# PacificBiosciences/trgt

Hardware: AMD Instinct MI355X
Metric: loci/s (higher is better)
Workload: dtype u8/u16 (WFA) + f64 (HMM); 1 GPU; BASELINE configs[1]: 10000 synthetic single-motif STR loci per GPU (motif 3-6 bp, allele <= 200 bp), 30 reads/locus HiFi-like, 10% truncated reads (SURVEY.md Appendix E), seed 20250509; contexts_per_gpu=4, loci_per_gpu=10000, reads_per_locus=30, parallelism=loci sharded across 1 GPU(s), no collective

## Files before the change

### trgt_amd/csrc/common.hpp

```cpp
#pragma once
#include <hip/hip_runtime.h>

#include <cstdarg>
#include <cstdint>
#include <cstdio>
#include <cstring>
#include <ctime>
#include <algorithm>
#include <mutex>
#include <string>
#include <vector>

#include "../../include/trgt_hip.h"

#ifdef TRGT_DEV_BUILD
#define TRGT_DEV_ENV(name) getenv(name)
#else
#define TRGT_DEV_ENV(name) ((const char*)nullptr)
#endif

struct trgt_knobs {
  int filter_force = 0;
  int flank_threads = 256;
  int heavy_band = 96;
  int heavy_threads = 0;
  int band_threads = 64;
  int win_threads = 64;
  int win_segments = 8;
  bool win_lds = false;
  bool band_lds = false;
  int grid_per_cu = 0;
  int filter_per_cu = 0;
  bool one_launch = false;
  bool no_spec = false;
  bool no_window = false;
  bool early_adaptive = true;
  bool no_heavy_window = false;
  bool no_sibling_rule = false;
  bool no_settled_sibling_rule = false;
  bool no_lcs_rule = false;
  bool no_indel_shortcut = false;
  bool no_hamming = false;
  bool no_filter = false;
  bool one_stream = false;
  bool host_genotyper = false;
  bool no_early = false;
  bool stage_lock = false;
  bool host_hmm_lists = false;
  bool debug = false;
  bool hmm_resolve_one_wg = false;
  bool wfa_no_wave_variant = false;
  bool wfa_no_stage = false;
  bool filter_side = false;
  bool filter_serial = false;
  bool filter_one_launch = false;
  bool no_long_window = false;
  bool no_long_filter = false;
  bool no_lean = false;
  bool lean_mid_tier = false;
  int lean_chunk = 0;
  bool no_zero_arena = false;
  bool hmm_ppl_per_class = false;
  bool hmm_ppl_wide = false;
  bool hmm_trace_wide = false;
  bool hmm_ppl_serial = false;
  bool lean_one_tier = false;
  bool no_lds_wfa = true;
  int lds_wfa_kb = 7;
  int lds_wfa_seq = 768;
  int sens_bialign_min_len = -1;
  bool sens_cons_unidir = false;
  bool sens_ward_ties = false;
  bool sens_lw_order = false;
  bool hmm_no_dedupe = false;
  bool hmm_no_long_tb = false;
  int hmm_long_wgs = 4;
  bool hmm_no_ppl = false;
  bool hmm_four_rounds = false;
  bool hmm_lds_fill = false;
  int cluster_arena_kb = 0;
  int repair_arena_kb = 0;
  bool host_cluster = false;
  bool host_purity = false;
  bool host_repair = false;
  bool split_hmm = false;
  int repair_blocks = 2048;
  int repair_max_seg = 0;
  bool timeline = false;
  bool skip_bt = false;
};

enum FlankRoute {
  FR_SIZE_TAG = 0,
  FR_SIZE_SNV,
  FR_CLUSTER_TAG,
  FR_CLUSTER_SNV,
  FR_CLUSTER_DEEP_TAG,
  FR_CLUSTER_DEEP_SNV,
  FR_N
};
struct FlankRouteState { bool on = false; int64_t stats[4] = {0, 0, 0, 0}; };

struct trgt_hip_ctx {
  trgt_knobs knobs;
  int device = -1;
  hipStream_t stream = nullptr;
  bool own_stream = false;
  int stream_priority = 0;
  bool in_pool = false;
  std::string err;
  uint64_t ws_limit = 32ull << 30;
  int32_t cluster_max_reads = 256;
  int32_t size_max_reads = 256;
  int64_t size_deep_stats[4] = {0, 0, 0, 0};
  FlankRouteState route[FR_N];
  double meth_ms[2] = {0, 0};
  double plot_ms[2] = {0, 0};
  int num_cus = 256;
  int band_occ = 0;
  struct Buf { void* p = nullptr; size_t cap = 0; };
  std::vector<Buf> pool;
  bool timing = false;
  double k_ms[TRGT_K_COUNT] = {};
  int64_t k_launches[TRGT_K_COUNT] = {};
  int64_t k_cells[TRGT_K_COUNT] = {};
  struct Pending { int k; hipEvent_t a, b; };
  std::vector<Pending> pending;
  std::vector<hipEvent_t> retired_events;
  void* zero_arena = nullptr; size_t zero_cap = 0, zero_used = 0, zero_dirty = 0; bool zero_on = false;
  void* wfa_cells_cur[3] = {nullptr, nullptr, nullptr};
  void* last_wfa_cells_dev = nullptr;
// ... 105 lines not shown
  S_HMM_EDIT, S_HMM_MAXD, S_HMM_PLEN, S_HMM_VISITS, S_HMM_LONG, S_HMM_MOTIFS,
  S_HMM_B_BASE, S_HMM_B_LAST = S_HMM_B_BASE + (S_HMM_MOTIFS - S_HMM_SEQ),
  S_WFA_SEQ, S_WFA_JOBS, S_WFA_WS, S_WFA_STATUS, S_WFA_SCORE, S_WFA_NMATCH, S_WFA_SPAN, S_WFA_CIGAR, S_WFA_CLEN, S_WFA_OPS,
  S_WFA_OLEN, S_WFA_COUNTER, S_WFA_CELLS, S_WFA_WS_B, S_WFA_COUNTER_B, S_WFA_CELLS_B, S_WFA_POFF, S_WFA_PACKED, S_WFA_RETRY, S_WFA_RETRY_B, S_WFA_WS_C, S_WFA_COUNTER_C, S_WFA_CELLS_C, S_WFA_RETRY_C, S_WFA_MID, S_WFA_MID_B, S_WFA_MID_C,
  S_FS_FLANK, S_FS_READS, S_FS_JOBS, S_FS_POS, S_FS_LIST, S_FS_COUNT, S_FS_OUT0, S_FS_OUT1, S_FS_HIT0, S_FS_HIT1,
  S_FS_WFAJOBS, S_FS_WFAJOBS_LONG, S_FS_KEEPJOBS, S_PF_READS0, S_PF_READS1, S_PF_FLANK0, S_PF_FLANK1, S_READS_PACKED, S_READS_EXPANDED, S_FLT_COUNTER, S_FLT_CELLS, S_FLT_COUNTER_B, S_FLT_CELLS_B, S_LW_FIRST, S_LW_SUB, S_LW_PARENT, S_LW_SUBKEEP, S_LW_JOBKEEP, S_LW_KEPT, S_LW_COUNT, S_FLT_SEQ, S_FLT_JOBS, S_FLT_SCORE, S_FLT_BOUND, S_FLT_KEEP, S_FS_WINJOBS, S_FS_RESTJOBS, S_FS_SCORE, S_FS_SPAN, S_FS_NMATCH, S_FS_HEAVY, S_FS_NOSEED, S_FS_BANDJOBS, S_FS_HRESTJOBS, S_FS_BSCORE, S_FS_LONGNOSEED, S_LW_SUBBAND, S_LW_JOBBEST, S_LW_JOBREJ, S_LW_BANDJOBS, S_LW_RESTJOBS, S_LW_BSCORE,
  S_LOCUS_0, S_LOCUS_1, S_LOCUS_2, S_LOCUS_3, S_LOCUS_4, S_LOCUS_5, S_LOCUS_6, S_LOCUS_7,
  S_GT_LRB, S_GT_PLOIDY, S_GT_TR, S_GT_TROFF, S_GT_TRLEN, S_GT_ALOFF, S_GT_ALCAP, S_GT_NEED, S_GT_NAL, S_GT_BLOB, S_GT_ALEN, S_GT_CI, S_GT_NSP,
  S_GT_CLS, S_GT_RANK, S_GT_NSPAN, S_GT_TOFF, S_GT_PACKED, S_GT_GENO,
  S_HMM_BUILD,
  S_VOTE_GROUPS, S_VOTE_SCRATCH, S_VOTE_OUT, S_VOTE_LEN,
  S_RP_GROUPS, S_RP_JOBS, S_RP_LOCI, S_RP_PEND, S_RP_CIGAR, S_RP_CLEN, S_RP_VOUT, S_RP_VLEN, S_RP_VSCR, S_RP_COUNTS,
  S_CL_LIST, S_CL_MOFF, S_CL_COUNTS, S_CL_REC, S_CL_CLS, S_CL_ESCORE, S_CL_GMAT, S_CL_EDJOBS, S_CL_JOBS, S_CL_GROUPS, S_CL_ED2JOBS, S_CL_ESCORE2, S_CL_CIGAR, S_CL_CLEN,
  S_CL_VOUT, S_CL_VLEN, S_CL_VSCR,
  S_INF_SRC, S_INF_DESC, S_INF_DST, S_INF_STATUS, S_INF_COUNTER,
  S_ZERO_ARENA,
  S_DEFL_SCRATCH,
  S_PUR_SLAB, S_PUR_CNT, S_PUR_RQ,
  S_CLD_LIST, S_CLD_LAST = S_CLD_LIST + (S_CL_VSCR - S_CL_LIST),
  S_CLD_SEL,
  S_GSD_LIST,
  S_GT_HP,
  S_SNV_SO, S_SNV_EO, S_SNV_MM, S_SNV_MMOFF, S_SNV_READ,
  S_SNV_DEEP,
  S_CLF_COUNTS,
  S_CLF_PEND,
  S_CLDF_COUNTS, S_CLDF_PEND,
  S_FS_SETTLED, S_FS_FILTERJOBS,
  S_FS_BANDFALL, S_LW_BANDFALL,
  S_METH_READS, S_METH_CALLS, S_METH_JOBS, S_METH_LOCI, S_METH_LEVEL, S_METH_LEN, S_METH_FLAG, S_METH_OUT, S_METH_NREADS, S_METH_PERREAD,
  S_PLOT_IN, S_PLOT_PATH, S_PLOT_HMMOUT, S_PLOT_WORK, S_PLOT_WFAOUT, S_PLOT_PSEG, S_PLOT_NPSEG, S_PLOT_RSEG, S_PLOT_NRSEG, S_PLOT_BPROJ, S_PLOT_SCORE, S_PLOT_POFF, S_PLOT_PACKED,
  S_COUNT
};
enum PinSlot { P_SPAN_S = 0, P_SPAN_E, P_HIT_L, P_HIT_R, P_CELLS, P_HMM_SEQ, P_HMM_SEQ_B, P_HMM_JOBS, P_HMM_JOBS_B, P_SEG0, P_SEG_META, P_GT_NEED, P_GT_NAL, P_GT_ALEN, P_GT_CI, P_GT_NSP, P_GT_CLS,
               P_GT_RANK, P_GT_NSPAN, P_GT_TOFF, P_GT_PACKED, P_HMM_BUILD, P_PUR_JOBS, P_COUNT };

inline int dev_get(trgt_hip_ctx* c, int slot, size_t bytes, void** out) {
  if ((int)c->pool.size() < S_COUNT) c->pool.resize(S_COUNT);
  auto& b = c->pool[slot];
  if (bytes == 0) bytes = 16;
  if (b.cap < bytes) {
    if (b.p) { TRGT_HIP_TRY(c, hipFree(b.p)); b.p = nullptr; b.cap = 0; }
    size_t want = bytes + bytes / 8 + 256;
    if (c->knobs.debug && want > ((size_t)256 << 20)) fprintf(stderr, "[mem] slot %d: %.2f GB\n", slot, (double)want / (double)(1ull << 30));
    if (want >= ((size_t)64 << 20)) {
      size_t free_b = 0, total_b = 0;
      if (hipMemGetInfo(&free_b, &total_b) == hipSuccess) {
        const size_t reserve = (size_t)1 << 30;
        if (free_b < want || free_b - want < reserve)
          return fail(c, TRGT_ERR_NOMEM, "%zu bytes of device memory wanted, %zu free: less than 1 GB would be left for the runtime (fewer contexts per GPU, or a smaller trgt_hip_set_workspace_limit)", want, free_b);
      } else (void)hipGetLastError();
    }
    hipError_t e = hipMalloc(&b.p, want);
    if (e != hipSuccess) {
      (void)hipGetLastError();
      b.p = nullptr;
      return fail(c, TRGT_ERR_NOMEM, "hipMalloc(%zu bytes) failed: %s", want, hipGetErrorString(e));
    }
    b.cap = want;
  }
  *out = b.p;
  return TRGT_OK;
}

inline int pin_get(trgt_hip_ctx* c, int slot, size_t bytes, void** out) {
  if ((int)c->pinned.size() < P_COUNT) c->pinned.resize(P_COUNT);
  auto& b = c->pinned[slot];
  if (bytes == 0) bytes = 16;
  if (b.cap < bytes) {
    if (b.p) { TRGT_HIP_TRY(c, hipHostFree(b.p)); b.p = nullptr; b.cap = 0; }
    const size_t want = bytes + bytes / 4 + 4096;
    hipError_t e = hipHostMalloc(&b.p, want, hipHostMallocDefault);
    if (e != hipSuccess) {
      (void)hipGetLastError();
      b.p = nullptr;
      return fail(c, TRGT_ERR_NOMEM, "hipHostMalloc(%zu bytes) failed: %s", want, hipGetErrorString(e));
    }
    b.cap = want;
  }
  *out = b.p;
  return TRGT_OK;
}

constexpr size_t ZERO_ARENA_BYTES = 2u << 20;
static __global__ void zero_arena_kernel(uint4* __restrict__ p, size_t n16) {
  for (size_t i = (size_t)blockIdx.x * blockDim.x + threadIdx.x; i < n16; i += (size_t)gridDim.x * blockDim.x) p[i] = make_uint4(0u, 0u, 0u, 0u);
}
inline int zero_begin(trgt_hip_ctx* c) {
  c->zero_on = false;
  if (c->knobs.no_zero_arena) return TRGT_OK;
  void* p = nullptr;
  if (int rc = dev_get(c, S_ZERO_ARENA, ZERO_ARENA_BYTES, &p)) return rc;
  const bool fresh = p != c->zero_arena;
  c->zero_arena = p; c->zero_cap = ZERO_ARENA_BYTES;
  const size_t dirty = fresh ? ZERO_ARENA_BYTES : std::min(ZERO_ARENA_BYTES, (std::max(c->zero_dirty, c->zero_used) + 4095) & ~(size_t)4095);
  if (dirty) {
    const size_t n16 = dirty / 16;
    hipLaunchKernelGGL(zero_arena_kernel, dim3((unsigned)std::min<size_t>(64, (n16 + 255) / 256)), dim3(256), 0, c->stream, (uint4*)p, n16);
    TRGT_HIP_TRY(c, hipGetLastError());
  }
  c->zero_used = 0; c->zero_dirty = 0; c->zero_on = true;
  c->wfa_cells_cur[0] = c->wfa_cells_cur[1] = c->wfa_cells_cur[2] = nullptr;
  return TRGT_OK;
}
inline void zero_end(trgt_hip_ctx* c) {
  if (c->zero_on) { c->zero_dirty = std::max(c->zero_dirty, c->zero_used); c->zero_on = false; }
  c->wfa_cells_cur[0] = c->wfa_cells_cur[1] = c->wfa_cells_cur[2] = nullptr;
}
inline void* zero_take(trgt_hip_ctx* c, size_t bytes) {
  if (!c->zero_on) return nullptr;
  const size_t need = (bytes + 63) & ~(size_t)63;
  if (c->zero_used + need > c->zero_cap) return nullptr;
  void* p = (uint8_t*)c->zero_arena + c->zero_used;
  c->zero_used += need;
  return p;
}
inline int dev_get_zeroed(trgt_hip_ctx* c, int slot, size_t bytes, void** out, hipStream_t stream) {
  if (void* z = zero_take(c, bytes)) { *out = z; return TRGT_OK; }
  if (int rc = dev_get(c, slot, bytes, out)) return rc;
  TRGT_HIP_TRY(c, hipMemsetAsync(*out, 0, bytes, stream));
  return TRGT_OK;
}

constexpr size_t H2D_KERNEL_MAX = 8u << 20;
static __global__ void h2d_copy_kernel(uint8_t* __restrict__ dst, const uint8_t* __restrict__ src, size_t bytes) {
  const size_t i = (size_t)blockIdx.x * blockDim.x + threadIdx.x, n = (size_t)gridDim.x * blockDim.x;
  if ((((uintptr_t)dst | (uintptr_t)src) & 15u) == 0) {
    const size_t n16 = bytes >> 4;
    for (size_t k = i; k < n16; k += n) reinterpret_cast<uint4*>(dst)[k] = reinterpret_cast<const uint4*>(src)[k];
    for (size_t k = (n16 << 4) + i; k < bytes; k += n) dst[k] = src[k];
  } else for (size_t k = i; k < bytes; k += n) dst[k] = src[k];
}
inline bool is_pinned_host_ptr(const void* p) {
  hipPointerAttribute_t at;
  if (hipPointerGetAttributes(&at, p) != hipSuccess) { (void)hipGetLastError(); return false; }
  return at.type == hipMemoryTypeHost;
}
inline int d2h(trgt_hip_ctx* c, void* dst, const void* src, size_t bytes, hipStream_t stream) {
  if (bytes == 0) return TRGT_OK;
  if (is_pinned_host_ptr(dst)) { TRGT_HIP_TRY(c, hipMemcpyAsync(dst, src, bytes, hipMemcpyDeviceToHost, stream)); return TRGT_OK; }
  const size_t need = (bytes + 63) & ~(size_t)63;
  trgt_hip_ctx::D2hChunk* ch = nullptr;
  for (auto& k : c->d2h_chunks) if (k.cap - k.used >= need) { ch = &k; break; }
  if (!ch) {
    trgt_hip_ctx::D2hChunk k;
    k.cap = std::max<size_t>(need, (size_t)4 << 20);
    if (hipHostMalloc(&k.p, k.cap, hipHostMallocDefault) != hipSuccess) { (void)hipGetLastError(); return fail(c, TRGT_ERR_NOMEM, "hipHostMalloc(%zu bytes) failed", k.cap); }
    c->d2h_chunks.push_back(k);
    ch = &c->d2h_chunks.back();
  }
  void* staged = (uint8_t*)ch->p + ch->used;
  ch->used += need;
  TRGT_HIP_TRY(c, hipMemcpyAsync(staged, src, bytes, hipMemcpyDeviceToHost, stream));
  c->d2h_pending.push_back({dst, staged, bytes, stream});
  return TRGT_OK;
}
inline hipError_t stream_wait(trgt_hip_ctx* c, hipStream_t stream) {
  const hipError_t e = stream_wait(stream);
  if (c->d2h_pending.empty()) return e;
  size_t kept = 0;
  for (auto& q : c->d2h_pending) {
    if (q.stream == stream) { if (e == hipSuccess) std::memcpy(q.dst, q.staged, q.bytes); }
    else c->d2h_pending[kept++] = q;
  }
  c->d2h_pending.resize(kept);
  if (kept == 0) {
// ... 178 lines not shown
```

### trgt_amd/csrc/ctx.hip

```cpp
#include "common.hpp"
#include "host_pool.hpp"

static std::string g_create_err;

#include <malloc.h>
static void tune_malloc_once() {
  static std::once_flag once;
  std::call_once(once, [] {
    const char* e = getenv("TRGT_MALLOC_TUNE");
    const int mode = e && *e ? atoi(e) : 1;
    if (mode <= 0) return;
    (void)mallopt(M_MMAP_THRESHOLD, 32 << 20);
    (void)mallopt(M_TRIM_THRESHOLD, 1 << 30);
    (void)mallopt(M_TOP_PAD, 64 << 20);
    if (mode >= 2) (void)mallopt(M_MMAP_MAX, 0);
  });
}

namespace trgt {
static thread_local int g_next_stream_priority = 0;
static thread_local bool g_next_in_pool = false;
void ctx_next_stream_priority(int p) { g_next_stream_priority = p; }
void ctx_next_in_pool(bool on) { g_next_in_pool = on; }
hipError_t make_stream(trgt_hip_ctx* c, hipStream_t* s) {
  return c->stream_priority ? hipStreamCreateWithPriority(s, hipStreamNonBlocking, c->stream_priority) : hipStreamCreateWithFlags(s, hipStreamNonBlocking);
}
hipError_t make_side_stream(trgt_hip_ctx* c, hipStream_t* s) {
  if (c->in_pool) return make_stream(c, s);
  int lo = 0, hi = 0;
  if (hipDeviceGetStreamPriorityRange(&lo, &hi) != hipSuccess || lo <= hi) { (void)hipGetLastError(); return make_stream(c, s); }
  const int base = c->stream_priority;
  const int side = base != hi ? hi : hi + 1;
  return hipStreamCreateWithPriority(s, hipStreamNonBlocking, side);
}
}

extern "C" {

int trgt_hip_abi_version(void) { return TRGT_HIP_ABI_VERSION; }

int trgt_hip_create(int device, trgt_hip_ctx** out) {
  if (!out) return TRGT_ERR_INVALID;
  *out = nullptr;
  int n = 0;
  hipError_t e = hipGetDeviceCount(&n);
  if (e != hipSuccess || n <= 0) {
    (void)hipGetLastError();
    g_create_err = "no HIP device visible (libtrgt_hip has no CPU fallback)";
    return TRGT_ERR_NO_DEVICE;
  }
  if (device < 0 || device >= n) { g_create_err = "device ordinal out of range"; return TRGT_ERR_INVALID; }
  e = hipSetDevice(device);
  if (e != hipSuccess) { g_create_err = hipGetErrorString(e); return TRGT_ERR_HIP; }
  hipDeviceProp_t prop;
  e = hipGetDeviceProperties(&prop, device);
  if (e != hipSuccess) { g_create_err = hipGetErrorString(e); return TRGT_ERR_HIP; }
  if (std::strncmp(prop.gcnArchName, "gfx950", 6) != 0) {
    g_create_err = std::string("device is ") + prop.gcnArchName + ", this library carries gfx950 code only";
    return TRGT_ERR_NO_DEVICE;
  }
  tune_malloc_once();
  trgt_hip_ctx* c = new trgt_hip_ctx();
  {
    trgt_knobs& k = c->knobs;
    auto num = [](const char* name, int dflt) { const char* e = getenv(name); return e && *e ? atoi(e) : dflt; };
    auto flag = [](const char* name) { const char* e = getenv(name); return e != nullptr && *e != 0 && std::strcmp(e, "0") != 0; };
#ifdef TRGT_DEV_BUILD
#define DEV_FLAG(name) flag(name)
#define DEV_NUM(name, dflt) num(name, dflt)
#else
#define DEV_FLAG(name) false
#define DEV_NUM(name, dflt) (dflt)
#endif
    (void)num; (void)flag;
    k.flank_threads = DEV_NUM("TRGT_FLANK_THREADS", k.flank_threads); k.heavy_threads = DEV_NUM("TRGT_HEAVY_THREADS", 0); k.heavy_band = std::max(0, std::min(num("TRGT_HEAVY_BAND", k.heavy_band), 256));
    k.win_threads = DEV_NUM("TRGT_WIN_THREADS", k.win_threads); { const int bt = DEV_NUM("TRGT_BAND_THREADS", k.band_threads); k.band_threads = bt == 128 || bt == 256 ? bt : 64; } k.win_segments = DEV_NUM("TRGT_WIN_SEGMENTS", k.win_segments); k.win_lds = DEV_FLAG("TRGT_WIN_LDS"); k.band_lds = DEV_FLAG("TRGT_BAND_LDS");
    k.grid_per_cu = DEV_NUM("TRGT_WFA_GRID_PER_CU", 0); k.filter_per_cu = DEV_NUM("TRGT_FILTER_PER_CU", 0);
    k.one_launch = DEV_FLAG("TRGT_WFA_ONE_LAUNCH"); k.no_spec = DEV_FLAG("TRGT_WFA_NO_SPEC"); k.no_window = flag("TRGT_WFA_NO_WINDOW"); k.no_hamming = flag("TRGT_NO_HAMMING"); k.no_indel_shortcut = flag("TRGT_NO_INDEL_SHORTCUT"); k.no_heavy_window = DEV_FLAG("TRGT_NO_HEAVY_WINDOW"); k.no_sibling_rule = DEV_FLAG("TRGT_NO_SIBLING_RULE"); k.no_settled_sibling_rule = DEV_FLAG("TRGT_NO_SETTLED_SIBLING_RULE"); k.no_lcs_rule = DEV_FLAG("TRGT_NO_LCS_RULE"); { const char* e = TRGT_DEV_ENV("TRGT_EARLY_ADAPTIVE"); if (e && *e) k.early_adaptive = std::strcmp(e, "0") != 0; }
    k.no_filter = flag("TRGT_WFA_NO_FILTER"); k.one_stream = DEV_FLAG("TRGT_FLANK_ONE_STREAM"); k.host_genotyper = flag("TRGT_HOST_GENOTYPER"); k.host_hmm_lists = DEV_FLAG("TRGT_HOST_HMM_LISTS"); k.no_early = flag("TRGT_WFA_NO_EARLY"); k.stage_lock = flag("TRGT_STAGE_LOCK"); k.no_long_filter = flag("TRGT_NO_LONG_FILTER"); k.no_long_window = DEV_FLAG("TRGT_NO_LONG_WINDOW"); k.filter_force = DEV_NUM("TRGT_FILTER_FORCE", 0); k.filter_one_launch = DEV_FLAG("TRGT_FILTER_ONE_LAUNCH"); k.filter_serial = DEV_FLAG("TRGT_FILTER_SERIAL"); k.filter_side = DEV_FLAG("TRGT_FILTER_SIDE"); k.wfa_no_stage = DEV_FLAG("TRGT_WFA_NO_STAGE"); k.wfa_no_wave_variant = DEV_FLAG("TRGT_WFA_NO_WAVE_VARIANT"); k.hmm_resolve_one_wg = DEV_FLAG("TRGT_HMM_RESOLVE_ONE_WG"); k.debug = flag("TRGT_WFA_DEBUG");
    k.timeline = flag("TRGT_TIMELINE");
    k.host_repair = flag("TRGT_HOST_REPAIR"); k.host_cluster = flag("TRGT_HOST_CLUSTER"); k.host_purity = DEV_FLAG("TRGT_HOST_PURITY"); k.cluster_arena_kb = num("TRGT_CLUSTER_ARENA_KB", 0); k.repair_arena_kb = num("TRGT_REPAIR_ARENA_KB", 0); k.hmm_lds_fill = DEV_FLAG("TRGT_HMM_LDS_FILL"); k.hmm_four_rounds = DEV_FLAG("TRGT_HMM_FOUR_ROUNDS"); k.hmm_no_ppl = flag("TRGT_HMM_NO_PPL"); k.hmm_long_wgs = std::max(1, std::min(DEV_NUM("TRGT_HMM_LONG_WGS", k.hmm_long_wgs), 16)); k.hmm_no_long_tb = flag("TRGT_HMM_NO_LONG_TB"); k.hmm_no_dedupe = flag("TRGT_HMM_NO_DEDUPE"); k.repair_max_seg = num("TRGT_REPAIR_MAX_SEG", k.repair_max_seg); k.split_hmm = DEV_FLAG("TRGT_SPLIT_HMM"); k.repair_blocks = DEV_NUM("TRGT_REPAIR_BLOCKS", k.repair_blocks);
    k.no_lean = flag("TRGT_WFA_NO_LEAN"); k.lean_one_tier = DEV_FLAG("TRGT_WFA_LEAN_ONE_TIER"); k.lean_mid_tier = DEV_FLAG("TRGT_WFA_LEAN_MID_TIER"); k.lean_chunk = DEV_NUM("TRGT_LEAN_CHUNK", 0); k.no_zero_arena = flag("TRGT_NO_ZERO_ARENA"); k.hmm_ppl_serial = DEV_FLAG("TRGT_HMM_PPL_SERIAL"); k.hmm_ppl_wide = DEV_FLAG("TRGT_HMM_PPL_WIDE"); k.hmm_trace_wide = DEV_FLAG("TRGT_HMM_TRACE_WIDE"); k.hmm_ppl_per_class = DEV_FLAG("TRGT_HMM_PPL_PER_CLASS");
    k.no_lds_wfa = !DEV_FLAG("TRGT_WFA_LDS"); k.lds_wfa_kb = DEV_NUM("TRGT_WFA_LDS_KB", k.lds_wfa_kb); k.lds_wfa_seq = DEV_NUM("TRGT_WFA_LDS_SEQ", k.lds_wfa_seq);
#ifdef TRGT_DEV_BUILD
    k.sens_bialign_min_len = num("TRGT_SENS_BIALIGN_MIN_LEN", -1); k.sens_cons_unidir = flag("TRGT_SENS_CONS_UNIDIR"); k.sens_ward_ties = flag("TRGT_SENS_WARD_TIES"); k.sens_lw_order = flag("TRGT_SENS_LW_ORDER");
    k.skip_bt = flag("TRGT_DBG_SKIP_BT");
#endif
  }
  c->device = device;
  c->num_cus = prop.multiProcessorCount;
  c->stream_priority = trgt::g_next_stream_priority;
  c->in_pool = trgt::g_next_in_pool;
  e = trgt::make_stream(c, &c->stream);
  if (e != hipSuccess) { g_create_err = hipGetErrorString(e); delete c; return TRGT_ERR_HIP; }
  c->own_stream = true;
  c->pool.resize(trgt::S_COUNT);
  *out = c;
  return TRGT_OK;
}

void trgt_hip_destroy(trgt_hip_ctx* c) {
  if (!c) return;
  (void)hipSetDevice(c->device);
  (void)trgt::stream_wait(c, c->stream);
  if (c->stream2) { (void)trgt::stream_wait(c, c->stream2); (void)hipStreamDestroy(c->stream2); }
  if (c->ev_upload) (void)hipEventDestroy(c->ev_upload);
  if (c->stream_copy) { (void)trgt::stream_wait(c, c->stream_copy); (void)hipStreamDestroy(c->stream_copy); }
  for (auto& st : c->staged) if (st.ready) (void)hipEventDestroy(st.ready);
  for (int i = 0; i < 6; ++i) {
    if (c->hmm_side[i]) { (void)trgt::stream_wait(c, c->hmm_side[i]); (void)hipStreamDestroy(c->hmm_side[i]); }
    if (c->hmm_join[i]) (void)hipEventDestroy(c->hmm_join[i]);
  }
  for (int i = 0; i < 2; ++i) if (c->hmm_fork[i]) (void)hipEventDestroy(c->hmm_fork[i]);
  for (int b = 0; b < 2; ++b)
    for (int k = 0; k < 4; ++k) {
      for (int g = 0; g < 3; ++g) {
        if (c->hmm_ppl_side[b][k][g]) { (void)trgt::stream_wait(c, c->hmm_ppl_side[b][k][g]); (void)hipStreamDestroy(c->hmm_ppl_side[b][k][g]); }
        if (c->hmm_ppl_join[b][k][g]) (void)hipEventDestroy(c->hmm_ppl_join[b][k][g]);
      }
      if (c->hmm_ppl_fork[b][k]) (void)hipEventDestroy(c->hmm_ppl_fork[b][k]);
    }
  if (c->ev_scan) (void)hipEventDestroy(c->ev_scan);
  if (c->ev_heavy) (void)hipEventDestroy(c->ev_heavy);
  if (c->ev_hwin) (void)hipEventDestroy(c->ev_hwin);
  if (c->stream_hmm) (void)hipStreamDestroy(c->stream_hmm);
  if (c->stream_flt) (void)hipStreamDestroy(c->stream_flt);
  if (c->ev_flt_a) (void)hipEventDestroy(c->ev_flt_a);
  if (c->ev_flt_b) (void)hipEventDestroy(c->ev_flt_b);
  if (c->ev_gt) (void)hipEventDestroy(c->ev_gt);
  if (c->ev_rp) (void)hipEventDestroy(c->ev_rp);
  delete static_cast<trgt::HostPool*>(c->host_pool);
  for (auto& b : c->h2d_stage) if (b.p) (void)hipHostFree(b.p);
  for (auto& k : c->d2h_chunks) if (k.p) (void)hipHostFree(k.p);
  for (auto& b : c->pinned)
    if (b.p) (void)hipHostFree(b.p);
  trgt::resolve_timing(c);
  for (auto& b : c->pool)
    if (b.p) (void)hipFree(b.p);
  trgt::resolve_timing(c);
  for (hipEvent_t e : c->retired_events) (void)hipEventDestroy(e);
  if (c->own_stream && c->stream) (void)hipStreamDestroy(c->stream);
  delete c;
}

const char* trgt_hip_last_error(const trgt_hip_ctx* c) { return c ? c->err.c_str() : g_create_err.c_str(); }

int trgt_hip_set_stream(trgt_hip_ctx* c, void* s) {
  if (!c) return TRGT_ERR_INVALID;
  (void)hipSetDevice(c->device);
  TRGT_HIP_TRY(c, trgt::stream_wait(c, c->stream));
  if (c->own_stream && c->stream) (void)hipStreamDestroy(c->stream);
  if (s == nullptr) {
    TRGT_HIP_TRY(c, trgt::make_stream(c, &c->stream));
    c->own_stream = true;
  } else {
    c->stream = (hipStream_t)s;
    c->own_stream = false;
  }
  return TRGT_OK;
// ... 38 lines not shown
```

### trgt_amd/csrc/hmm.hip

```cpp
#include <algorithm>
#include <type_traits>
#include <cmath>
#include <limits>
#include <thread>

#include "common.hpp"

namespace trgt {


}
#include <memory>

#include "hmm_host.hpp"
namespace trgt {

struct HmmJobDev {
  uint32_t set, seq_len, job_index, path_cap;
  uint64_t seq_off, bp_off, path_off, span_off, count_off, visit_off;
  uint64_t map_off;
};

static inline uint64_t align_up(uint64_t v, uint64_t a) { return (v + a - 1) / a * a; }

// ... 1332 lines not shown
#pragma unroll
  for (int c = 1; c < HMM_SLOT_CLASSES; ++c) k += i >= a.class_begin[c] ? 1u : 0u;
  return k;
}
__global__ void __launch_bounds__(256) hmm_resolve_count_kernel(const HmmResolveAllArgs a) {
  const uint32_t i = blockIdx.x * 256u + threadIdx.x;
  const int lane = (int)(threadIdx.x & 63u);
  uint32_t v = 0, key = 0;
  if (i < a.n) {
    const uint32_t slot = a.cand[i].job_index, l = slot >> 1, al = slot & 1u;
    const bool on = !a.skip_locus[l] && (int32_t)al < a.n_alleles[l];
    if (!on) { a.n_spans[slot] = 0; a.purity[slot] = __builtin_nan(""); }
    v = on ? a.allele_len[slot] + 1u : 0u;
    if (a.dup) {
      uint8_t d = 0;
      if (on && al == 1u && i > 0 && a.cand[i - 1].job_index == slot - 1u && a.allele_len[slot - 1u] == a.allele_len[slot]) {
        const uint8_t* p = a.seq_blob + a.cand[i - 1].seq_off; const uint8_t* q = a.seq_blob + a.cand[i].seq_off;
        const uint32_t n = a.allele_len[slot];
        uint64_t diff = 0;
        uint32_t t = 0;
        for (; t + 8 <= n; t += 8) { uint64_t x, y; __builtin_memcpy(&x, p + t, 8); __builtin_memcpy(&y, q + t, 8); diff |= x ^ y; }
        for (; t < n; ++t) diff |= (uint64_t)(p[t] ^ q[t]);
        d = diff == 0 ? 1 : 0;
      }
      a.dup[i] = d;
      if (d) v = 0;
    }
    a.verdict[i] = v;
    if (v) { const uint32_t b = (v - 1u) >> a.len_shift; key = hmm_class_of(a, i) * 64u + (63u - (b < 63u ? b : 63u)); }
  }
  uint32_t rank, count, leader;
  hmm_wave_keys(v != 0u, key, lane, rank, count, leader);
  if (v && rank == 0u) atomicAdd(&a.hist[key], count);
}
__global__ void __launch_bounds__(256) hmm_resolve_scatter_kernel(const HmmResolveAllArgs a) {
  __shared__ uint32_t base[HMM_RESOLVE_KEYS];
  for (uint32_t t = threadIdx.x; t < (uint32_t)HMM_RESOLVE_KEYS; t += 256) base[t] = a.hist[t];
  __syncthreads();
  if (threadIdx.x < (uint32_t)HMM_SLOT_CLASSES) {
    uint32_t run = 0;
    for (int b = 0; b < 64; ++b) { const uint32_t h = base[threadIdx.x * 64 + b]; base[threadIdx.x * 64 + b] = run; run += h; }
    if (blockIdx.x == 0) a.n_jobs[threadIdx.x] = run;
  }
  __syncthreads();
  const uint32_t i = blockIdx.x * 256u + threadIdx.x;
  const int lane = (int)(threadIdx.x & 63u);
  const uint32_t v = i < a.n ? a.verdict[i] : 0u;
  uint32_t key = 0, k = 0;
  if (v) { k = hmm_class_of(a, i); const uint32_t b = (v - 1u) >> a.len_shift; key = k * 64u + (63u - (b < 63u ? b : 63u)); }
  uint32_t rank, count, leader;
  hmm_wave_keys(v != 0u, key, lane, rank, count, leader);
  uint32_t at = 0;
  if (v && rank == 0u) at = atomicAdd(&a.taken[key], count);
  at = (uint32_t)__shfl((int)at, (int)leader);
  if (!v) return;
  HmmJobDev jd = a.cand[i];
  jd.seq_len = v - 1u;
  a.jobs[a.class_begin[k] + base[key] + at + rank] = jd;
}

__global__ void __launch_bounds__(256) hmm_dup_copy_kernel(const HmmJobDev* __restrict__ cand, uint32_t n, const uint8_t* __restrict__ dup, const HmmSetDev* __restrict__ sets,
                                                           int32_t* __restrict__ spans3, uint32_t* __restrict__ n_spans, uint32_t* __restrict__ counts, double* __restrict__ purity) {
  const uint32_t i = blockIdx.x * 256u + threadIdx.x;
  if (i >= n || !dup[i]) return;
  const HmmJobDev a = cand[i - 1], b = cand[i];
  const uint32_t ns = n_spans[a.job_index];
  n_spans[b.job_index] = ns; purity[b.job_index] = purity[a.job_index];
  for (uint32_t k = 0; k < 3 * ns; ++k) spans3[3 * b.span_off + k] = spans3[3 * a.span_off + k];
  const uint32_t nm = sets[b.set].n_blocks - 1;
  for (uint32_t k = 0; k < nm; ++k) counts[b.count_off + k] = counts[a.count_off + k];
}

__global__ void hmm_pack_spans_kernel(const int32_t* __restrict__ spans3, const uint64_t* __restrict__ job_span_off,
                                      const uint32_t* __restrict__ n_spans, const uint64_t* __restrict__ packed_off,
                                      int32_t* __restrict__ packed, uint64_t n_jobs) {
  const uint64_t j = (uint64_t)blockIdx.x * blockDim.x + threadIdx.x;
  if (j >= n_jobs) return;
  const int32_t* src = spans3 + 3 * job_span_off[j];
  int32_t* dst = packed + 3 * packed_off[j];
  for (uint32_t i = 0; i < 3 * n_spans[j]; ++i) dst[i] = src[i];
}

__global__ void __launch_bounds__(1024) hmm_span_prefix_kernel(const uint32_t* __restrict__ n_spans, uint64_t* __restrict__ off, uint64_t n) {
  __shared__ uint64_t part[1024];
  const uint32_t t = threadIdx.x;
  const uint64_t per = (n + 1023) / 1024, b = t * per < n ? t * per : n, e = b + per < n ? b + per : n;
  uint64_t sum = 0;
  for (uint64_t i = b; i < e; ++i) sum += n_spans[i];
  part[t] = sum;
  __syncthreads();
  if (t == 0) { uint64_t run = 0; for (int i = 0; i < 1024; ++i) { const uint64_t v = part[i]; part[i] = run; run += v; } off[n] = run; }
  __syncthreads();
  uint64_t run = part[t];
  for (uint64_t i = b; i < e; ++i) { off[i] = run; run += n_spans[i]; }
}


#include "hmm_batch.hpp"

}

using namespace trgt;

extern "C" uint64_t trgt_hmm_path_capacity(uint32_t seq_len, uint32_t max_motif_len) {
  if (seq_len == 0) return 1;
  return (uint64_t)(seq_len + 2) * (max_motif_len + 4) + 8;
}

extern "C" int trgt_hmm_models_check(trgt_hip_ctx* c, int32_t n_sets, const uint8_t* motif_blob, const uint32_t* motif_off,
                                     const uint32_t* set_motif_begin, int64_t* n_diff) {
  if (!c || !n_diff) return TRGT_ERR_INVALID;
  *n_diff = -1;
  HmmModels dev, host;
  int rc = hmm_models_on_device(c, n_sets, motif_blob, motif_off, set_motif_begin, dev, c->stream, nullptr);
  if (rc) return fail(c, rc, "%s", dev.err.empty() ? trgt_hip_last_error(c) : dev.err.c_str());
  rc = hmm_build_models(n_sets, motif_blob, motif_off, set_motif_begin, host);
  if (rc) return fail(c, rc, "%s", host.err.c_str());
  std::vector<uint8_t> got((size_t)dev.blob_bytes);
  if (dev.blob_bytes) { const int d2h_rc = trgt::d2h(c, got.data(), dev.d_blob, (size_t)dev.blob_bytes, c->stream); if (d2h_rc) return d2h_rc; }
  TRGT_HIP_TRY(c, trgt::stream_wait(c, c->stream));
  int64_t diff = dev.blob_bytes > host.blob.size() ? (int64_t)(dev.blob_bytes - host.blob.size()) : (int64_t)(host.blob.size() - dev.blob_bytes);
  const size_t n = std::min((size_t)dev.blob_bytes, host.blob.size());
  for (size_t i = 0; i < n; ++i) diff += got[i] != host.blob[i];
  const uint8_t *a = (const uint8_t*)dev.sets.data(), *b = (const uint8_t*)host.sets.data();
  for (size_t i = 0; i < sizeof(HmmSetDev) * (size_t)n_sets; ++i) diff += a[i] != b[i];
  *n_diff = diff;
  return TRGT_OK;
}

extern "C" int trgt_hmm_batch(trgt_hip_ctx* c, int32_t n_sets, const uint8_t* motif_blob, const uint32_t* motif_off,
                              const uint32_t* set_motif_begin, int64_t n_jobs, const uint32_t* job_set,
                              const uint8_t* seq_blob, const uint64_t* seq_off, const uint32_t* seq_len, uint16_t* path,
                              const uint64_t* path_off, uint32_t* path_len, int32_t* spans3, const uint64_t* span_off,
                              uint32_t* n_spans, uint32_t* motif_counts, const uint64_t* count_off, double* purity,
                              int32_t* edit_dist, int32_t* max_dist) {
  HmmBatchIO io;
  io.n_sets = n_sets; io.motif_blob = motif_blob; io.motif_off = motif_off; io.set_motif_begin = set_motif_begin;
  io.n_jobs = n_jobs; io.job_set = job_set; io.seq_blob = seq_blob; io.seq_off = seq_off; io.seq_len = seq_len;
  io.path = path; io.path_off = path_off; io.path_len = path_len; io.spans3 = spans3; io.span_off = span_off; io.n_spans = n_spans;
  io.motif_counts = motif_counts; io.count_off = count_off; io.purity = purity; io.edit_dist = edit_dist; io.max_dist = max_dist;
  return hmm_batch_impl(c, nullptr, io);
}
```

### trgt_amd/csrc/locus.hip

```cpp
#include <algorithm>
#include <array>
#include <chrono>
#include <cmath>
#include <cstddef>
#include <cstdlib>
#include <functional>
#include <optional>
#include <thread>

#include "hmm_host.hpp"
#include "host_pool.hpp"
#include "locus_gt.hpp"
#include "locus_purity.hpp"
#include "locus_cluster_dev.hpp"
#include "locus_cluster_deep.hpp"
#include "locus_cluster_flank.hpp"
#include "locus_gt_deep.hpp"
#include "locus_cluster_flank_deep.hpp"
#include "wfa_host.hpp"

namespace trgt {

namespace {

// ... 337 lines not shown
      }
      if (nc && (x != m_len[j] || y != bb_len[g])) return fail(c, TRGT_ERR_INVALID, "trgt_dev_consensus_vote: CIGAR of member %llu ends at (%llu, %llu), not at (%u, %u)", (unsigned long long)j, (unsigned long long)x, (unsigned long long)y, m_len[j], bb_len[g]);
      JobDev& jd = jobs[(size_t)j];
      jd.pat_off = bb_off[g]; jd.pat_len = bb_len[g]; jd.txt_off = m_off[j]; jd.txt_len = m_len[j]; jd.cigar_off = slot_words; jd.ops_off = 0; jd.out_index = (uint32_t)j; jd.pad = 0;
      po[(size_t)j] = bb_off[g]; pl[(size_t)j] = bb_len[g]; clen[(size_t)j] = (uint32_t)nc;
      slot_words += (uint64_t)bb_len[g] + m_len[j] + 1;
    }
  }
  first[(size_t)n_groups] = n_members;
  std::vector<uint32_t> slots((size_t)slot_words, 0xFFFFFFFFu);
  for (size_t j = 0; j < n_members; ++j) std::copy(cigar + cigar_first[j], cigar + cigar_first[j + 1], slots.begin() + (ptrdiff_t)jobs[j].cigar_off);
  int rc;
  void *d_seq = nullptr, *d_jobs = nullptr, *d_cig = nullptr, *d_clen = nullptr;
  if ((rc = dev_get(c, S_WFA_SEQ, (size_t)seq_bytes + 16, &d_seq)) || (rc = dev_get(c, S_WFA_JOBS, n_members * sizeof(JobDev), &d_jobs)) ||
      (rc = dev_get(c, S_WFA_CIGAR, (size_t)slot_words * 4 + 16, &d_cig)) || (rc = dev_get(c, S_WFA_CLEN, n_members * 4, &d_clen)))
    return rc;
  TRGT_HIP_TRY(c, hipMemcpyAsync(d_seq, seqs, (size_t)seq_bytes, hipMemcpyHostToDevice, c->stream));
  TRGT_HIP_TRY(c, hipMemcpyAsync(d_jobs, jobs.data(), n_members * sizeof(JobDev), hipMemcpyHostToDevice, c->stream));
  TRGT_HIP_TRY(c, hipMemcpyAsync(d_cig, slots.data(), (size_t)slot_words * 4, hipMemcpyHostToDevice, c->stream));
  TRGT_HIP_TRY(c, hipMemcpyAsync(d_clen, clen.data(), n_members * 4, hipMemcpyHostToDevice, c->stream));
  TRGT_HIP_TRY(c, trgt::stream_wait(c, c->stream));
  WfaOnDevice dev;
  dev.jobs = (const JobDev*)d_jobs; dev.cigar = (const uint32_t*)d_cig; dev.cigar_len = (const uint32_t*)d_clen; dev.seqs = (const uint8_t*)d_seq;
  std::vector<vote::Group> groups;
  std::vector<uint32_t> lens;
  std::vector<uint8_t> bytes;
  if ((rc = vote_groups(c, dev, po.data(), pl.data(), m_len, first, out_cap, count_on_device != 0, 0, groups, lens, bytes))) return rc;
  for (int64_t g = 0; g < n_groups; ++g) {
    out_len[g] = lens[(size_t)g];
    if (lens[(size_t)g] == 0xFFFFFFFFu) continue;
    const uint64_t room = out_off[g + 1] - out_off[g];
    std::memcpy(out_bytes + out_off[g], bytes.data() + groups[(size_t)g].out_off, (size_t)std::min<uint64_t>(room, lens[(size_t)g]));
  }
  return TRGT_OK;
}
#endif

#include "locus_cluster.hpp"

__global__ void repair_check_kernel(const gt::RepairBufs rp, uint64_t read_bytes) {
  const uint32_t nj = rp.counts[gt::RC_JOBS], ng = rp.counts[gt::RC_GROUPS];
  for (uint32_t j = blockIdx.x * blockDim.x + threadIdx.x; j < nj; j += gridDim.x * blockDim.x) {
    const JobDev jd = rp.jobs[j];
    const bool bad = jd.pat_len > rp.max_seg || jd.txt_len > rp.max_seg || jd.pat_off + jd.pat_len > read_bytes || jd.txt_off + jd.txt_len > read_bytes ||
                     jd.cigar_off + jd.pat_len + jd.txt_len + 1 > rp.cap_cigar || jd.out_index != j;
    if (bad) { atomicAdd(rp.counts + 10, 1u); rp.counts[11] = j; rp.counts[12] = jd.pat_len; rp.counts[13] = jd.txt_len; rp.counts[14] = jd.out_index; rp.counts[15] = (uint32_t)jd.cigar_off; }
  }
  if (blockIdx.x == 0 && threadIdx.x == 0 && (nj > rp.cap_jobs || ng > rp.cap_groups)) atomicAdd(rp.counts + 10, 1000000u);
}

static uint32_t* g_trace_dump = nullptr;
static uint32_t* repair_trace_buf() {
  if (!TRGT_DEV_ENV("TRGT_REPAIR_TRACE")) return nullptr;
  if (!g_trace_dump) (void)hipHostMalloc((void**)&g_trace_dump, 4096, hipHostMallocDefault);
  return g_trace_dump;
}
__global__ void repair_trace_kernel(const gt::RepairBufs rp, uint32_t* host) {
  if (threadIdx.x < gt::RC_WORDS) host[threadIdx.x] = __hip_atomic_load(rp.counts + threadIdx.x, __ATOMIC_RELAXED, __HIP_MEMORY_SCOPE_AGENT);
  if (threadIdx.x < 8) { const JobDev jd = rp.jobs[threadIdx.x]; uint32_t* h = host + 16 + 8 * threadIdx.x;
    h[0] = (uint32_t)jd.pat_off; h[1] = jd.pat_len; h[2] = (uint32_t)jd.txt_off; h[3] = jd.txt_len; h[4] = (uint32_t)jd.cigar_off; h[5] = jd.out_index; h[6] = (uint32_t)(jd.pat_off >> 32); h[7] = (uint32_t)(jd.txt_off >> 32); }
  __threadfence_system();
}
__global__ void zero_words_kernel(uint32_t* p, uint32_t n) { for (uint32_t i = threadIdx.x; i < n; i += blockDim.x) atomicExch(p + i, 0u); }

struct GatherArgs { const uint8_t* reads; const uint64_t* src_off; const uint64_t* dst_off; const uint32_t* len; uint64_t n; uint8_t* out; };
__global__ void gather_segments_kernel(const GatherArgs a) {
  const uint64_t s = (uint64_t)blockIdx.x * 4 + (threadIdx.x >> 6);
  if (s >= a.n) return;
  const uint8_t* __restrict__ src = a.reads + a.src_off[s];
  uint8_t* __restrict__ dst = a.out + a.dst_off[s];
  for (uint32_t i = threadIdx.x & 63; i < a.len[s]; i += 64) dst[i] = src[i];
}

inline int64_t now_ns() { return std::chrono::duration_cast<std::chrono::nanoseconds>(std::chrono::steady_clock::now().time_since_epoch()).count(); }

HostPool* host_pool(trgt_hip_ctx* c, int threads) {
  if (c->host_pool && c->host_pool_threads != threads) { delete static_cast<HostPool*>(c->host_pool); c->host_pool = nullptr; }
  if (!c->host_pool) { c->host_pool = new HostPool(threads); c->host_pool_threads = threads; }
  return static_cast<HostPool*>(c->host_pool);
}

struct CountCopy { const uint32_t* src1; uint32_t* dst1; uint32_t n1; const uint32_t* src2; uint32_t* dst2; uint32_t n2; const uint32_t* src3; uint32_t* dst3; uint32_t n3; };
__global__ void __launch_bounds__(1024) allele_prefix_kernel(const uint32_t* __restrict__ len, uint64_t* __restrict__ off, int64_t n, const CountCopy cc) {
  __shared__ uint64_t part[1024];
  const int t = threadIdx.x;
  if ((uint32_t)t < cc.n1) cc.dst1[t] = cc.src1 ? __hip_atomic_load(cc.src1 + t, __ATOMIC_RELAXED, __HIP_MEMORY_SCOPE_AGENT) : 0u;
  if ((uint32_t)t < cc.n2) cc.dst2[t] = cc.src2 ? __hip_atomic_load(cc.src2 + t, __ATOMIC_RELAXED, __HIP_MEMORY_SCOPE_AGENT) : 0u;
  if ((uint32_t)t < cc.n3) cc.dst3[t] = cc.src3 ? __hip_atomic_load(cc.src3 + t, __ATOMIC_RELAXED, __HIP_MEMORY_SCOPE_AGENT) : 0u;
  const int64_t per = (n + 1023) / 1024, b = t * per, e = b + per < n ? b + per : n;
  uint64_t sum = 0;
  for (int64_t i = b; i < e; ++i) sum += len[i];
  part[t] = sum;
  __syncthreads();
  if (t == 0) { uint64_t run = 0; for (int i = 0; i < 1024; ++i) { const uint64_t v = part[i]; part[i] = run; run += v; } off[n] = run; }
  __syncthreads();
  uint64_t run = part[t];
  for (int64_t i = b; i < e; ++i) { off[i] = run; run += len[i]; }
}
__global__ void allele_pack_kernel(const uint8_t* __restrict__ blob, const uint64_t* __restrict__ src_off, const uint32_t* __restrict__ len,
                                   const uint64_t* __restrict__ dst_off, uint8_t* __restrict__ packed, int64_t n) {
  const int64_t i = (int64_t)blockIdx.x * 4 + (threadIdx.x >> 6);
  if (i >= n) return;
  const uint8_t* s = blob + src_off[i];
  uint8_t* d = packed + dst_off[i];
  for (uint32_t b = threadIdx.x & 63; b < len[i]; b += 64) d[b] = s[b];
}

}
}

using namespace trgt;

extern "C" int32_t trgt_median_i32(const int32_t* data, int64_t n, float* out) {
  if (n < 0 || (n > 0 && !data) || !out) return TRGT_ERR_INVALID;
  if (n == 0) return 0;
  try { std::vector<int32_t> v(data, data + n); *out = median_f32(v); return 1; } catch (const std::exception&) { return TRGT_ERR_NOMEM; }
}

extern "C" void trgt_locus_default_params(trgt_locus_params* p) {
  if (!p) return;
  std::memset(p, 0, sizeof *p);
  p->flank_len = 250; p->min_flank_id_frac = 0.7; p->max_depth = 250; p->mism = 2; p->gapo = 5; p->gape = 1; p->host_threads = 0;
  p->min_read_qual = 0.98;
}

static std::mutex g_upload_mutex[16];
static hipStream_t g_upload_stream[16];
static hipStream_t bulk_upload_stream(trgt_hip_ctx* c) {
  static const bool shared = [] { const char* e = TRGT_DEV_ENV("TRGT_SHARED_UPLOAD_STREAM"); return !(e && *e == '0'); }();
  if (!shared) return c->stream_copy;
  const size_t d = (size_t)c->device % 16;
  if (!g_upload_stream[d] && hipStreamCreateWithFlags(&g_upload_stream[d], hipStreamNonBlocking) != hipSuccess) { (void)hipGetLastError(); return c->stream_copy; }
  return g_upload_stream[d];
}
static int issue_pending_uploads(trgt_hip_ctx* c) {
  bool any = false;
  for (auto& st : c->staged) any = any || (st.in_use && st.copy_pending);
  if (!any) return TRGT_OK;
  std::lock_guard<std::mutex> upload_lock(g_upload_mutex[(size_t)c->device % 16]);
  const hipStream_t up = bulk_upload_stream(c);
  for (auto& st : c->staged) {
    if (!st.in_use || !st.copy_pending) continue;
    st.copy_pending = false;
    if (st.d_reads) {
      static const size_t piece = [] { const char* e = TRGT_DEV_ENV("TRGT_UPLOAD_CHUNK_MB"); const long v = e && *e ? atol(e) : 32; return v > 0 ? (size_t)v << 20 : (size_t)0; }();
      const size_t total = (size_t)st.read_bytes;
      static const int kernel_wgs = [] { const char* e = TRGT_DEV_ENV("TRGT_UPLOAD_KERNEL"); return e && *e ? atoi(e) : 0; }();
      if (kernel_wgs > 0 && is_pinned_host_ptr(st.in->read_blob)) {
        hipLaunchKernelGGL(h2d_copy_kernel, dim3((unsigned)kernel_wgs), dim3(256), 0, up, const_cast<uint8_t*>(st.d_reads), st.in->read_blob, total);
        TRGT_HIP_TRY(c, hipGetLastError());
      } else
      for (size_t o = 0; o < total; o += piece ? piece : total) {
        const size_t n = piece ? std::min(piece, total - o) : total;
        TRGT_HIP_TRY(c, hipMemcpyAsync(const_cast<uint8_t*>(st.d_reads) + o, st.in->read_blob + o, n, hipMemcpyHostToDevice, up));
      }
    }
    if (st.d_flank) TRGT_HIP_TRY(c, hipMemcpyAsync(const_cast<uint8_t*>(st.d_flank), st.in->flank_blob, (size_t)st.flank_bytes, hipMemcpyHostToDevice, up));
    TRGT_HIP_TRY(c, hipEventRecord(st.ready, up));
  }
  return TRGT_OK;
}

static std::mutex g_stage_a_mutex[16];

__device__ __forceinline__ uint32_t bam4_pair_to_ascii(uint32_t b) {
  const uint64_t lo = 0x565352474d43413dull , hi = 0x4e42444b48595754ull ;
  const uint32_t a = b >> 4, z = b & 15u;
  const uint32_t ca = (uint32_t)(((a & 8u) ? hi : lo) >> (8 * (a & 7u))) & 0xFFu, cz = (uint32_t)(((z & 8u) ? hi : lo) >> (8 * (z & 7u))) & 0xFFu;
  return ca | (cz << 8);
}
__global__ void __launch_bounds__(256) expand_bam4_kernel(const uint8_t* __restrict__ packed, uint8_t* __restrict__ out, uint64_t n_bytes) {
  const uint64_t n16 = n_bytes / 16;
  for (uint64_t i = (uint64_t)blockIdx.x * blockDim.x + threadIdx.x; i < n16; i += (uint64_t)gridDim.x * blockDim.x) {
    const uint4 v = ((const uint4*)packed)[i];
    const uint32_t w[4] = {v.x, v.y, v.z, v.w};
    uint32_t o[8];
#pragma unroll
    for (int k = 0; k < 4; ++k) {
      o[2 * k] = bam4_pair_to_ascii(w[k] & 0xFFu) | (bam4_pair_to_ascii((w[k] >> 8) & 0xFFu) << 16);
      o[2 * k + 1] = bam4_pair_to_ascii((w[k] >> 16) & 0xFFu) | (bam4_pair_to_ascii(w[k] >> 24) << 16);
// ... 72 lines not shown

  trgt_hip_ctx* const c; const trgt_locus_params* const p; const trgt_locus_batch_in* in; trgt_locus_batch_out* const out;
  const uint8_t *staged_reads, *staged_flank; const hipEvent_t ready;
  const int64_t nl; int64_t nr = 0; int F = 0;
  bool done = false;
  trgt_locus_batch_in in_expanded; std::vector<uint64_t> expanded_off;
  bool reads_on_device = false, impure_filter = false, dev_gt = false, presel = false, flank_on = false, use_slots = false, dev_repair = false, split = false, small_gt = false;
  FlankMeta flank_meta{};
  bool zeroed = false;
  HmmPending *hmm_pending = nullptr, *hmm_pending2 = nullptr, *hmm_pendingB = nullptr;
  hipEvent_t evA = nullptr;
  std::unique_lock<std::mutex> stage_a_token;
  std::optional<StreamGuard> host_streams;
  HostPool* pool = nullptr;
  std::vector<uint64_t> piece_off; std::vector<uint32_t> read_locus, heavy_len;
  uint64_t flank_total = 0, read_total = 0, tr_total = 0, allele_total = 0, max_locus_reads = 0; uint32_t max_read_len = 0, heavy_tlen_max = 0;
  UploadBatch ub;
  const uint8_t *d_flank = nullptr, *d_reads = nullptr; const uint64_t *d_piece = nullptr, *d_roff = nullptr; const uint32_t *d_rlen = nullptr, *d_rloc = nullptr, *d_heavy = nullptr;
  void *d_ss = nullptr, *d_se = nullptr, *d_hl = nullptr, *d_hr = nullptr, *h_ss = nullptr, *h_se = nullptr, *h_hl = nullptr, *h_hr = nullptr, *h_cells = nullptr;
  Slab slab;
  size_t o_ss = 0, o_se = 0, o_hl = 0, o_hr = 0, o_need = 0, o_nal = 0, o_alen = 0, o_ci = 0, o_nsp = 0, o_cls = 0, o_rank = 0, o_nspan = 0, o_toff = 0, o_flip = 0, o_gsz = 0,
         o_rpc = 0, o_skipb = 0, o_clc = 0, o_cldc = 0, o_fdone = 0, o_cfc = 0, o_cfdc = 0;
  GtDev g; GtHost gh;
  ClPlan clp[2];
  std::vector<uint32_t>& cl_list = clp[0].list; std::vector<uint32_t>& cld_list = clp[1].list;
  uint32_t cld_no_room = 0;
  std::vector<uint32_t> gsd_list; const uint32_t* d_gsd_list = nullptr;
  gt::GtArgs ga; RepairDev rb;
  const uint32_t* cl_counts_dev[2] = {nullptr, nullptr};
  cld::DeepArgs da, ds;
  HmmModels models; HmmSlots hs;
  HmmBatchIO hmm_io(uint32_t* n_spans, double* purity) const {
    HmmBatchIO io;
    io.n_sets = (int32_t)nl; io.motif_blob = in->motif_blob; io.motif_off = in->motif_off; io.set_motif_begin = in->set_motif_begin;
    io.spans3 = out->spans3; io.span_off = out->span_off; io.n_spans = n_spans; io.motif_counts = out->motif_counts; io.count_off = out->count_off; io.purity = purity;
    return io;
  }
  HmmBatchIO hmm_list_io(const std::vector<uint32_t>& set, const void* blob, const std::vector<uint64_t>& off, const std::vector<uint32_t>& len, uint32_t* n_spans, double* purity) const {
    HmmBatchIO io = hmm_io(n_spans, purity);
    io.n_jobs = (int64_t)set.size(); io.job_set = set.data(); io.seq_blob = (const uint8_t*)blob; io.seq_off = off.data(); io.seq_len = len.data();
    return io;
  }
  hipStream_t upload_stream = nullptr;
  std::vector<uint8_t> slot_skip;
  std::vector<uint32_t> nsB; std::vector<double> puB;
  std::vector<uint32_t> job_set, seq_len, nsp; std::vector<uint64_t> seq_off, span_off, count_off; std::vector<int64_t> slot; std::vector<double> pur;
  std::vector<uint32_t> js2, sl2, ns2; std::vector<uint64_t> so2, spo2, co2; std::vector<double> pu2; std::vector<int64_t> slot2;
  bool outputs_ready = false;
  bool published = false, hmm1_done = false;
  std::vector<int64_t> R; int64_t nR = 0;
  std::vector<uint8_t> need_a;
  const int32_t *sp_s = nullptr, *sp_e = nullptr;
  std::vector<LocusWork> work; std::vector<uint64_t> sel_begin; std::vector<K> sel; std::vector<uint32_t> n_sel; std::vector<Scratch> scratch;
  std::vector<uint64_t> seg_src, seg_dst; std::vector<uint32_t> seg_len, seg_read; std::vector<const uint8_t*> seg_ptr;
  uint64_t n_seg = 0, seg_bytes = 0; void* h_seg = nullptr;
  std::vector<ClusterLocus> cl_loci; std::vector<std::vector<Seg>> cl_trs; std::vector<FlankRes> fres;
  bool tl_on = false;
  int64_t t0 = 0, tA = 0, tB = 0, tC = 0, tHost = 0, tw_a = 0, th_begin = 0, th0 = 0;
  int64_t stat_flank_jobs = 0, stat_flank_heavy = 0, stat_cons_jobs = 0, stat_spanning = 0, stat_hmm_jobs = 0, stat_ed_jobs = 0;

  LocusCall(trgt_hip_ctx* c_, const trgt_locus_params* p_, const trgt_locus_batch_in* in_, trgt_locus_batch_out* out_, const uint8_t* staged_reads_,
            const uint8_t* staged_flank_, hipEvent_t ready_)
      : c(c_), p(p_), in(in_), out(out_), staged_reads(staged_reads_), staged_flank(staged_flank_), ready(ready_), nl(in_->n_loci),
        stage_a_token(g_stage_a_mutex[(size_t)c_->device % 16], std::defer_lock), ub(c_, c_->stream) {}
  ~LocusCall() {
    host_streams.reset();
    if (stage_a_token.owns_lock()) stage_a_token.unlock();
    if (evA) (void)hipEventDestroy(evA);
    for (HmmPending* q : {hmm_pendingB, hmm_pending2, hmm_pending}) if (q) hmm_pending_free(q);
    if (zeroed) trgt::zero_end(c);
  }

  bool is_cluster(int64_t l) const { return in->genotyper && in->genotyper[l] == 1; }
  bool fits[FR_N] = {}, ran[FR_N] = {};
  void plan_routes();
  bool any_route_fits() const { return std::any_of(fits, fits + FR_N, [](bool b) { return b; }); }
  bool cluster_route_fits() const { return fits[FR_CLUSTER_TAG] || fits[FR_CLUSTER_SNV]; }
  bool deep_cluster_route_fits() const { return fits[FR_CLUSTER_DEEP_TAG] || fits[FR_CLUSTER_DEEP_SNV]; }
  bool snv_inputs_up() const { return fits[FR_SIZE_SNV] || fits[FR_CLUSTER_SNV] || fits[FR_CLUSTER_DEEP_SNV]; }
  bool tags_up() const { return fits[FR_SIZE_TAG] || fits[FR_CLUSTER_TAG] || fits[FR_CLUSTER_DEEP_TAG] || (snv_inputs_up() && in->hp_tag); }
  enum class GtForm { PLAIN, FLANK, SNV };
  GtForm gt_form() const { return fits[FR_SIZE_SNV] ? GtForm::SNV : fits[FR_SIZE_TAG] ? GtForm::FLANK : GtForm::PLAIN; }
  void launch_genotype_kernels(), launch_finish_kernels(const gt::FinishArgs& fa);
  void tally_route(FlankRoute r, const std::vector<uint32_t>* list, uint8_t snv, const uint8_t* fdone, const uint8_t* need);
  gt::GtFlankArgs flank_args() const { gt::GtFlankArgs fa; static_cast<gt::GtArgs&>(fa) = ga; fa.hp_tag = g.hp; fa.flank_done = (uint8_t*)slab.d(o_fdone); return fa; }
  gt::SnvArgs snv_args() const {
    gt::SnvArgs sa; static_cast<gt::GtFlankArgs&>(sa) = flank_args();
    sa.start_offset = g.so; sa.end_offset = g.eo; sa.mismatch_offsets = g.mm; sa.mismatch_off = g.mm_off; sa.snv_read = (uint8_t*)g.snv_read;
    sa.ln_match = std::log(0.9); sa.ln_mis = std::log(1.0 - 0.9); sa.ln2 = std::log(2.0); sa.tag_route = fits[FR_SIZE_TAG] ? 1 : 0;
    return sa;
  }
  gtd::DeepFlankArgs deep_flank_args() const { return gtd::DeepFlankArgs{ds, g.hp, (uint8_t*)slab.d(o_fdone)}; }
  gtd::DeepSnvArgs deep_snv_args() const {
    gtd::DeepSnvArgs da; static_cast<gtd::DeepFlankArgs&>(da) = deep_flank_args();
    const gt::SnvArgs sa = snv_args();
    da.start_offset = sa.start_offset; da.end_offset = sa.end_offset; da.mismatch_offsets = sa.mismatch_offsets; da.mismatch_off = sa.mismatch_off; da.snv_read = sa.snv_read;
    da.ln_match = sa.ln_match; da.ln_mis = sa.ln_mis; da.ln2 = sa.ln2; da.tag_route = sa.tag_route;
    da.prof = (uint64_t*)g.snv_prof; da.stage = (int32_t*)g.snv_stage; da.stage_cap = in->mismatch_off[nr];
    return da;
  }
  uint64_t& cell(int w) { return ((uint64_t*)h_cells)[w]; }
  void tl(const char* name) const { if (tl_on) fprintf(stderr, "[tl] %-28s %7.2f ms  ctx=%p\n", name, (double)(now_ns() - t0) / 1e6, (void*)c); }

  int check_args(), host_tables(), upload_tables(), plan_device_lists(), flush_uploads(), locate_flanks();
  int repair_buffers(), purity_chain(), size_genotyper(), repair_chain(), cluster_chain(int deep), enqueue_results();
  int wait_stage_a(), gather_host_segments(), host_front(), host_flank(), host_back(), host_stage_c(), collect_all();
  void stage_c_job_lists(), select_host_reads();
  void init_outputs();
  int collect_ab(), collect_hmm1(), hmm1_enqueue(), hmm1_once(), publish();
};
int LocusCall::check_args() {
  if (nl < 0) return fail(c, TRGT_ERR_INVALID, "trgt_locus_batch: negative n_loci");
  for (int64_t& v : c->size_deep_stats) v = 0;
  for (FlankRouteState& r : c->route) for (int64_t& v : r.stats) v = 0;
  if (nl == 0) { done = true; return TRGT_OK; }
  if (!in->flank_blob || !in->lf_off || !in->lf_len || !in->rf_off || !in->rf_len || !in->tr_blob || !in->tr_off || !in->tr_len ||
      !in->motif_blob || !in->motif_off || !in->set_motif_begin || !in->ploidy || !in->locus_read_begin || !in->read_blob ||
      !in->read_off || !in->read_len || !out->span_start || !out->span_end || !out->n_alleles || !out->allele_blob ||
      !out->allele_off || !out->allele_cap || !out->allele_len || !out->ci || !out->num_spanning || !out->classification ||
      !out->read_rank || !out->spans3 || !out->span_off || !out->n_spans || !out->motif_counts || !out->count_off || !out->purity)
    return fail(c, TRGT_ERR_INVALID, "trgt_locus_batch: null field");
  TRGT_HIP_TRY(c, hipSetDevice(c->device));
  zeroed = true;
  { const int zrc = trgt::zero_begin(c); if (zrc) return zrc; }
  F = p->flank_len;
  if (F <= 0) return fail(c, TRGT_ERR_INVALID, "trgt_locus_batch: flank_len must be positive");
  nr = (int64_t)in->locus_read_begin[nl];
  if (2 * nr > 0xFFFFFFF0ll) return fail(c, TRGT_ERR_UNSUPPORTED, "trgt_locus_batch: too many reads in one call");
  if (in->read_encoding != TRGT_READS_ASCII && in->read_encoding != TRGT_READS_BAM4) return fail(c, TRGT_ERR_INVALID, "trgt_locus_batch: read_encoding %d", in->read_encoding);
  if (in->read_encoding == TRGT_READS_BAM4 && nr > 0) {
    uint64_t packed_total = 0;
    expanded_off.resize((size_t)nr);
    for (int64_t r = 0; r < nr; ++r) {
      packed_total = std::max<uint64_t>(packed_total, in->read_off[r] + ((uint64_t)in->read_len[r] + 1) / 2);
      expanded_off[(size_t)r] = 2 * in->read_off[r];
    }
    const uint8_t* d_packed = nullptr;
    void* d_exp = nullptr;
    int erc;
    if (ready) TRGT_HIP_TRY(c, hipStreamWaitEvent(c->stream, ready, 0));
    if (staged_reads) d_packed = staged_reads;
    else if ((erc = dev_in(c, S_READS_PACKED, in->read_blob, (size_t)packed_total, &d_packed))) return erc;
    if ((erc = dev_get(c, S_READS_EXPANDED, 2 * (size_t)packed_total + 64, &d_exp))) return erc;
    const unsigned blocks = (unsigned)std::min<uint64_t>((uint64_t)c->num_cus * 16, packed_total / (16 * 256) + 1);
    hipLaunchKernelGGL(expand_bam4_kernel, dim3(blocks), dim3(256), 0, c->stream, d_packed, (uint8_t*)d_exp, packed_total);
    TRGT_HIP_TRY(c, hipGetLastError());
    in_expanded = *in;
    in_expanded.read_blob = (const uint8_t*)d_exp; in_expanded.read_off = expanded_off.data(); in_expanded.read_encoding = TRGT_READS_ASCII;
    in = &in_expanded;
    staged_reads = nullptr;
  }
  return TRGT_OK;
}
void LocusCall::init_outputs() {
  for (int64_t l = 0; l < nl; ++l) {
    out->n_alleles[l] = 0; out->allele_len[2 * l] = out->allele_len[2 * l + 1] = 0; out->num_spanning[2 * l] = out->num_spanning[2 * l + 1] = 0;
    if (out->gt_size) out->gt_size[2 * l] = out->gt_size[2 * l + 1] = 0;
    if (out->flipped) out->flipped[l] = 0;
  }
  for (int64_t r = 0; r < nr; ++r) { out->classification[r] = -1; out->read_rank[r] = -1; out->span_start[r] = out->span_end[r] = -1; }
  for (int64_t s = 0; s < 2 * nl; ++s) { out->n_spans[s] = 0; out->purity[s] = std::nan(""); }
}
int LocusCall::host_tables() {
  int threads = p->host_threads > 0 ? p->host_threads : (int)std::max(1u, std::thread::hardware_concurrency());
  threads = std::min(threads, !c->knobs.host_genotyper && !(p->min_read_qual < 0.9 && c->knobs.host_purity) ? 8 : 32);
  pool = host_pool(c, threads);
// ... 262 lines not shown
    da.c.g = ga; da.purity_on = 1; da.read_qual = pa.read_qual; da.pj_counter = pa.counter; da.pj = pa.jobs; da.pj_cap = pa.cap_jobs; da.purity = pa.purity;
    hipLaunchKernelGGL(cld::deep_select_kernel, dim3(da.c.n_list), dim3(cld::DW), 0, c->stream, da);
  }
  if (!gsd_list.empty()) {
    ds.c.g = ga; ds.purity_on = 1; ds.read_qual = pa.read_qual; ds.pj_counter = pa.counter; ds.pj = pa.jobs; ds.pj_cap = pa.cap_jobs; ds.purity = pa.purity;
    hipLaunchKernelGGL(cld::deep_select_kernel, dim3(ds.c.n_list), dim3(cld::DW), 0, c->stream, ds);
  }
  TRGT_HIP_TRY(c, hipGetLastError());
  *(uint32_t*)h_pj = 0;
  { const int d2h_rc = trgt::d2h(c, h_pj, pa.counter, 4, c->stream); if (d2h_rc) return d2h_rc; }
  tl_mark(c, "purity selection enqueued");
  init_outputs(); outputs_ready = true;
  const int64_t tw_p = now_ns();
  TRGT_HIP_TRY(c, trgt::stream_wait(c, c->stream));
  tA += now_ns() - tw_p;
  tl("purity jobs listed");
  const int64_t n_pj = (int64_t)std::min<uint32_t>(*(const uint32_t*)h_pj, pa.cap_jobs);
  if (n_pj > 0) {
    const pur::PurityJob* pj = pa.jobs;
    std::vector<uint32_t> pj_set((size_t)n_pj), pj_len((size_t)n_pj); std::vector<uint64_t> pj_off((size_t)n_pj), pj_cnt_off((size_t)n_pj);
    uint64_t cnt_total = 0;
    for (int64_t j = 0; j < n_pj; ++j) {
      if ((int64_t)pj[j].locus >= nl) return fail(c, TRGT_ERR_INVALID, "trgt_locus_batch: purity job %lld names locus %u", (long long)j, pj[j].locus);
      pj_set[(size_t)j] = pj[j].locus; pj_off[(size_t)j] = pj[j].seq_off; pj_len[(size_t)j] = pj[j].seq_len;
      pj_cnt_off[(size_t)j] = cnt_total; cnt_total += in->set_motif_begin[pj[j].locus + 1] - in->set_motif_begin[pj[j].locus];
    }
    void* d_pcnt = nullptr;
    if ((rc = dev_get(c, S_PUR_CNT, ((size_t)cnt_total + 1) * 4, &d_pcnt))) return rc;
    const int64_t tc0 = now_ns();
    HmmBatchIO io = hmm_list_io(pj_set, d_reads, pj_off, pj_len, (uint32_t*)ps.d(po_nsp), (double*)ps.d(po_pur));
    io.spans3 = nullptr; io.span_off = nullptr; io.motif_counts = (uint32_t*)d_pcnt; io.count_off = pj_cnt_off.data();
    rc = hmm_batch_impl(c, &models, io);
    if (rc) return rc;
    tC += now_ns() - tc0;
    stat_hmm_jobs += n_pj;
    tl("purity batch done");
  }
  k_purity_filter.launch(!small_gt, true, pgrid, c->stream, ga, pa);
  if (!cld_list.empty()) hipLaunchKernelGGL(cld::deep_filter_kernel, dim3(da.c.n_list), dim3(cld::DW), 0, c->stream, da);
  if (!gsd_list.empty()) hipLaunchKernelGGL(cld::deep_filter_kernel, dim3(ds.c.n_list), dim3(cld::DW), 0, c->stream, ds);
  TRGT_HIP_TRY(c, hipGetLastError());
  ga.sel_read = pa.sel_read; ga.sel_start = pa.sel_start; ga.sel_len = pa.sel_len; ga.n_sel = pa.n_sel;
  return TRGT_OK;
}
void LocusCall::launch_genotype_kernels() {
  const bool deep = !gsd_list.empty();
  const dim3 grid((unsigned)nl), dgrid(ds.c.n_list), dblock(cld::DW);
  if (deep) ds.c.g = ga;
  auto select = [&] { if (!presel) hipLaunchKernelGGL(cld::deep_select_kernel, dgrid, dblock, 0, c->stream, ds); };
  switch (gt_form()) {
    case GtForm::SNV:
      k_genotype_snv.launch(!small_gt, presel, grid, c->stream, snv_args());
      if (deep) { select(); hipLaunchKernelGGL((gtd::deep_size_genotype_kernel<true, true>), dgrid, dblock, 0, c->stream, deep_snv_args()); }
      break;
    case GtForm::FLANK:
      k_genotype_flank.launch(!small_gt, presel, grid, c->stream, flank_args());
      if (deep) { select(); hipLaunchKernelGGL(gtd::deep_size_genotype_kernel<true>, dgrid, dblock, 0, c->stream, deep_flank_args()); }
      break;
    case GtForm::PLAIN:
      k_genotype.launch(!small_gt, presel, grid, c->stream, ga);
      if (deep) { select(); hipLaunchKernelGGL(gtd::deep_size_genotype_kernel<false>, dgrid, dblock, 0, c->stream, ds); }
      break;
  }
}
void LocusCall::launch_finish_kernels(const gt::FinishArgs& fa) {
  const bool deep = !gsd_list.empty();
  const dim3 grid((unsigned)nl), dgrid(ds.c.n_list), dblock(cld::DW);
  if (deep) ds.c.g = ga;
  switch (gt_form()) {
    case GtForm::SNV:
      k_repair_finish_snv.launch(!small_gt, presel, grid, c->stream, snv_args(), fa);
      if (deep) hipLaunchKernelGGL((gtd::deep_size_finish_kernel<true, true>), dgrid, dblock, 0, c->stream, deep_snv_args(), fa);
      break;
    case GtForm::FLANK:
      k_repair_finish_flank.launch(!small_gt, presel, grid, c->stream, flank_args(), fa);
      if (deep) hipLaunchKernelGGL(gtd::deep_size_finish_kernel<true>, dgrid, dblock, 0, c->stream, deep_flank_args(), fa);
      break;
    case GtForm::PLAIN:
      k_repair_finish.launch(!small_gt, presel, grid, c->stream, ga, fa);
      if (deep) hipLaunchKernelGGL(gtd::deep_size_finish_kernel<false>, dgrid, dblock, 0, c->stream, ds, fa);
      break;
  }
}
int LocusCall::size_genotyper() {
  if (!dev_gt) return TRGT_OK;
  launch_genotype_kernels();
  ran[FR_SIZE_TAG] = fits[FR_SIZE_TAG]; ran[FR_SIZE_SNV] = fits[FR_SIZE_SNV];
  TRGT_HIP_TRY(c, hipGetLastError());
  tl_mark(c, "genotyper launched");
  split = use_slots && dev_repair && c->knobs.split_hmm;
  ga.finish_clears_need = split ? 0 : 1;
  if (use_slots && split) {
    if (!c->ev_gt) TRGT_HIP_TRY(c, hipEventCreateWithFlags(&c->ev_gt, hipEventDisableTiming));
    if (!c->ev_rp) TRGT_HIP_TRY(c, hipEventCreateWithFlags(&c->ev_rp, hipEventDisableTiming));
    if (!c->stream_hmm) TRGT_HIP_TRY(c, trgt::make_side_stream(c, &c->stream_hmm));
    TRGT_HIP_TRY(c, hipEventRecord(c->ev_gt, c->stream));
  }
  if (use_slots && split) {
    int rc; int64_t tc0;
    {
      StreamGuard keep(c);
      TRGT_HIP_TRY(c, hipStreamWaitEvent(c->stream_hmm, c->ev_gt, 0)); TRGT_HIP_TRY(c, hipStreamWaitEvent(c->stream_hmm, c->ev_upload, 0)); c->stream = c->stream_hmm;
      hs.d_skip = (const uint8_t*)g.need;
      tc0 = now_ns();
      rc = hmm_enqueue_slots(c, &models, hs, hmm_io(out->n_spans, out->purity), &hmm_pending);
    }
    if (rc) return rc;
    tC += now_ns() - tc0;
    tl("hmm1 enqueued (device-resolved job list)");
  }
  return TRGT_OK;
}
int LocusCall::repair_chain() {
  if (!dev_gt || !dev_repair) return TRGT_OK;
  int rc;
  gt::RepairBufs& rp = ga.rp;
  StreamGuard keep(c);
  if (split) {
    TRGT_HIP_TRY(c, hipStreamWaitEvent(c->stream2, c->ev_gt, 0));
    std::swap(c->stream, c->stream2);
  }
  trgt_wfa_params wp;
  trgt_wfa_default_params(&wp);
  wp.metric = 3; wp.mismatch = 2; wp.gap_open1 = 5; wp.gap_ext1 = 1; wp.span = 0; wp.scope = 1; wp.memory_mode = 3; sens_apply(c, wp);
  WfaLaunch LR;
  LR.jobs_dev = rp.jobs; LR.n_jobs_host = (int64_t)std::min<uint64_t>(rp.cap_jobs, (uint64_t)std::max(64, c->knobs.repair_blocks)); LR.n_jobs_dev = rp.counts + gt::RC_JOBS; LR.jobs_bound = rp.cap_jobs;
  LR.pat_base = d_reads; LR.txt_base = d_reads;
  LR.max_plen = rp.max_seg; LR.max_tlen = rp.max_seg; LR.max_sum = 2 * (int64_t)rp.max_seg;
  LR.cigar = (uint32_t*)rb.cig; LR.cigar_len = (uint32_t*)rb.clen; LR.buffer_set = 2; LR.ws_budget = 512ull << 20; LR.refused = rp.counts + gt::RC_REFUSED;
  auto dbg_sync = [&](const char* what) -> int {
    if (!c->knobs.debug) return TRGT_OK;
    const hipError_t e = trgt::stream_wait(c, c->stream);
    uint32_t h[gt::RC_WORDS]; std::memset(h, 0, sizeof h);
    if (e == hipSuccess) (void)hipMemcpy(h, rp.counts, sizeof h, hipMemcpyDeviceToHost);
    fprintf(stderr, "[repair] %s: %s (groups %u jobs %u loci %u failed %u cigar words %llu)\n", what, hipGetErrorString(e), h[gt::RC_GROUPS], h[gt::RC_JOBS], h[gt::RC_LOCI], h[gt::RC_FAILED],
            (unsigned long long)h[gt::RC_CIGAR] | ((unsigned long long)h[gt::RC_CIGAR + 1] << 32));
    return e == hipSuccess ? TRGT_OK : fail(c, TRGT_ERR_HIP, "%s failed: %s", what, hipGetErrorString(e));
  };
  if ((rc = dbg_sync("genotyper"))) return rc;
  if (uint32_t* trace_host = repair_trace_buf()) { std::memset(trace_host, 0, 4096); hipLaunchKernelGGL(repair_trace_kernel, dim3(1), dim3(64), 0, c->stream, rp, trace_host); }
  static const bool repair_check = TRGT_DEV_ENV("TRGT_REPAIR_CHECK") != nullptr;
  if (repair_check) {
    hipLaunchKernelGGL(repair_check_kernel, dim3(64), dim3(256), 0, c->stream, rp, (uint64_t)read_total);
    uint32_t h[gt::RC_WORDS];
    (void)trgt::stream_wait(c, c->stream);
    (void)hipMemcpy(h, rp.counts, sizeof h, hipMemcpyDeviceToHost);
    fprintf(stderr, "[repair check] jobs %u groups %u loci %u bad %u (last bad job %u: plen %u tlen %u out_index %u cigar_off %u) caps: jobs %u cigar %llu max_seg %u read bytes %llu\n", h[1], h[0], h[2], h[10], h[11], h[12], h[13],
            h[14], h[15], rp.cap_jobs, (unsigned long long)rp.cap_cigar, rp.max_seg, (unsigned long long)read_total);
  }
  if ((rc = wfa_launch(c, wp, LR))) return rc;
  if ((rc = dbg_sync("consensus alignments"))) return rc;
  vote::VoteArgs va{(const vote::Group*)rp.groups, 0u, rp.counts + gt::RC_GROUPS, d_reads, rp.jobs, (const uint32_t*)rb.cig, (const uint32_t*)rb.clen,
                    (uint32_t*)rb.vscr, (uint8_t*)rb.vout, (uint32_t*)rb.vlen};
  hipLaunchKernelGGL(vote::consensus_vote_kernel, dim3((unsigned)rp.cap_groups), dim3(vote::VOTE_THREADS), 0, c->stream, va);
  const gt::FinishArgs fa{(const uint8_t*)rb.vout, (const uint32_t*)rb.vlen};
  launch_finish_kernels(fa);
  TRGT_HIP_TRY(c, hipGetLastError());
  if ((rc = dbg_sync("vote + finish"))) return rc;
  tl_mark(c, "repair chain enqueued");
  if (split) {
    TRGT_HIP_TRY(c, hipEventRecord(c->ev_rp, c->stream));
    hs.d_skip = (const uint8_t*)slab.d(o_skipb);
    nsB.assign(2 * (size_t)nl, 0); puB.assign(2 * (size_t)nl, 0.0);
    const int64_t tc0 = now_ns();
    if ((rc = hmm_enqueue_slots(c, &models, hs, hmm_io(nsB.data(), puB.data()), &hmm_pendingB, 1))) return rc;
    tC += now_ns() - tc0;
    std::swap(c->stream, c->stream2);
    TRGT_HIP_TRY(c, hipStreamWaitEvent(c->stream, c->ev_rp, 0));
  }
  return TRGT_OK;
}
int LocusCall::cluster_chain(int deep) {
  if (!dev_gt || clp[deep].list.empty()) return TRGT_OK;
  int rc;
  const uint64_t cl_pairs = clp[deep].pairs, cl_reads = clp[deep].reads;
  const uint32_t n_cl = (uint32_t)clp[deep].list.size();
  const uint32_t max_seg = max_read_len > 2u * (uint32_t)F ? max_read_len - 2u * (uint32_t)F : 1u;
  cl::ClArgs ca;
  std::memset(&ca, 0, sizeof ca);
  ca.g = ga; ca.list = clp[deep].d_list; ca.n_list = n_cl; ca.mat_off = clp[deep].d_moff;
  ca.flags = (c->knobs.sens_ward_ties ? 1u : 0u) | (c->knobs.sens_lw_order ? 2u : 0u);
  ca.cap_j = (uint32_t)cl_reads; ca.cap_g = 2 * n_cl; ca.vote_lds_pos = (uint32_t)vote::VOTE_LDS_POS;
  const bool snv_route = !deep && fits[FR_CLUSTER_SNV];
  const bool route = !deep && cluster_route_fits();
  const bool deep_snv_route = deep && fits[FR_CLUSTER_DEEP_SNV];
  const bool deep_route = deep && deep_cluster_route_fits();
  if (deep) { ran[FR_CLUSTER_DEEP_TAG] = fits[FR_CLUSTER_DEEP_TAG]; ran[FR_CLUSTER_DEEP_SNV] = fits[FR_CLUSTER_DEEP_SNV]; }
  else { ran[FR_CLUSTER_TAG] = fits[FR_CLUSTER_TAG]; ran[FR_CLUSTER_SNV] = fits[FR_CLUSTER_SNV]; }
  const uint64_t rounds = (snv_route || deep_snv_route) ? 4 : (route || deep_route) ? 3 : 2;
  ca.cap_cigar = std::min<uint64_t>(rounds * cl_reads * (2ull * max_seg + 1), 96ull << 20);
  ca.cap_out = std::min<uint64_t>(rounds * (cl_reads + 2ull * n_cl) * ((uint64_t)max_seg + 16) + 64, 256ull << 20);
  ca.cap_scratch = std::min<uint64_t>(3ull * rounds * cl_reads + 6ull * rounds * n_cl * ((uint64_t)max_seg + 1) + 64, 32ull << 20);
  if (c->knobs.cluster_arena_kb > 0) {
    const uint64_t kb = (uint64_t)c->knobs.cluster_arena_kb;
    ca.cap_cigar = std::min<uint64_t>(ca.cap_cigar, kb * 256); ca.cap_out = std::min<uint64_t>(ca.cap_out, kb * 1024); ca.cap_scratch = std::min<uint64_t>(ca.cap_scratch, kb * 256);
  }
  const bool big = clp[deep].max_nr > 64;
  void *d_cnt = nullptr, *d_rec = nullptr, *d_cls = nullptr, *d_es = nullptr, *d_gm = nullptr, *d_edj = nullptr, *d_j = nullptr, *d_g = nullptr, *d_ed2 = nullptr, *d_es2 = nullptr,
       *d_cig = nullptr, *d_clen = nullptr, *d_vout = nullptr, *d_vlen = nullptr, *d_vscr = nullptr;
  if ((rc = dev_get(c, cl_slot(deep, S_CL_COUNTS), 256, &d_cnt)) || (rc = dev_get(c, cl_slot(deep, S_CL_REC), (size_t)n_cl * sizeof(cl::ClRec), &d_rec)) || (rc = dev_get(c, cl_slot(deep, S_CL_CLS), (size_t)nr + 16, &d_cls)) ||
      (rc = dev_get(c, cl_slot(deep, S_CL_ESCORE), (size_t)cl_pairs * 4 + 16, &d_es)) || (big && (rc = dev_get(c, cl_slot(deep, S_CL_GMAT), (size_t)cl_pairs * 8 + 16, &d_gm))) ||
      (rc = dev_get(c, cl_slot(deep, S_CL_EDJOBS), (size_t)cl_pairs * sizeof(JobDev) + 16, &d_edj)) || (rc = dev_get(c, cl_slot(deep, S_CL_JOBS), (size_t)rounds * ca.cap_j * sizeof(JobDev), &d_j)) ||
      (rc = dev_get(c, cl_slot(deep, S_CL_GROUPS), (size_t)rounds * ca.cap_g * sizeof(gt::RGroup), &d_g)) || (rc = dev_get(c, cl_slot(deep, S_CL_ED2JOBS), 2 * (size_t)cl_reads * sizeof(JobDev), &d_ed2)) ||
      (rc = dev_get(c, cl_slot(deep, S_CL_ESCORE2), 2 * (size_t)nr * 4 + 16, &d_es2)) || (rc = dev_get(c, cl_slot(deep, S_CL_CIGAR), (size_t)ca.cap_cigar * 4, &d_cig)) ||
      (rc = dev_get(c, cl_slot(deep, S_CL_CLEN), (size_t)rounds * ca.cap_j * 4, &d_clen)) || (rc = dev_get(c, cl_slot(deep, S_CL_VOUT), (size_t)ca.cap_out + 16, &d_vout)) ||
      (rc = dev_get(c, cl_slot(deep, S_CL_VLEN), (size_t)rounds * ca.cap_g * 4, &d_vlen)) || (rc = dev_get(c, cl_slot(deep, S_CL_VSCR), (size_t)ca.cap_scratch * 4 + 16, &d_vscr)))
    return rc;
  void* const z_clc = zero_take(c, 256);
  ca.counts = z_clc ? (uint32_t*)z_clc : (uint32_t*)d_cnt; ca.rec = (cl::ClRec*)d_rec; ca.cls = (int8_t*)d_cls; ca.escore = (int32_t*)d_es; ca.gmat = (double*)d_gm;
  ca.ed_jobs = (JobDev*)d_edj; ca.jobs = (JobDev*)d_j; ca.groups = (gt::RGroup*)d_g; ca.ed2_jobs = (JobDev*)d_ed2; ca.escore2 = (int32_t*)d_es2;
  ca.vote_out = (const uint8_t*)d_vout; ca.vote_len = (const uint32_t*)d_vlen;
  if (!z_clc) hipLaunchKernelGGL(zero_words_kernel, dim3(1), dim3(64), 0, c->stream, ca.counts, (uint32_t)cl::CC_WORDS);
  const dim3 cgrid(n_cl);
  auto step = [&](void (*deep_kernel)(cld::DeepArgs), const OneWave<cl::ClArgs>& shallow) {
    if (deep) hipLaunchKernelGGL(deep_kernel, cgrid, dim3(cld::DW), 0, c->stream, da);
    else shallow.launch(big, presel, cgrid, c->stream, ca);
  };
  if (deep) {
    da.c = ca;
    if (!presel) hipLaunchKernelGGL(cld::deep_select_kernel, cgrid, dim3(cld::DW), 0, c->stream, da);
  }
  step(cld::deep_front_kernel, k_cluster_front);
// ... 984 lines not shown
```

### trgt_amd/csrc/locus_gt.hpp

```cpp
#pragma once
#include <type_traits>

#include "common.hpp"
#include "repair_queue.hpp"

namespace trgt {
namespace gt {

constexpr int GT_MAX_READS = 256;
constexpr int GT_SEG_LDS = 16 * 1024;

constexpr int32_t RP_FLANK = 0x100;
constexpr int32_t RP_SNV = 0x200;
enum { FL_DONE = 1, FL_REPAIRED = 2, FL_HANDED = 4, FL_NOSPLIT = 8, FL_SNV = 16, FL_UNDECIDED = 32 };
constexpr int SNV_MAX_SNVS = 64;
constexpr int SNV_MAX_HAPS = 16;
constexpr int SNV_OFFS_PER_READ = 8;
enum { SR_ASSIGN = 1, SR_IN0 = 2, SR_IN1 = 4 };

struct GtArgs {
  const uint8_t* reads; const uint64_t* read_off; const uint32_t* read_len; const uint64_t* locus_read_begin;
  const int32_t* span_start; const int32_t* span_end;
  const uint8_t* ploidy; const uint8_t* tr_blob; const uint64_t* tr_off; const uint32_t* tr_len;
  const uint64_t* allele_off; const uint32_t* allele_cap;
  int64_t n_loci; int32_t flank_len, max_depth;
  uint8_t* need_host; int32_t* n_alleles; uint8_t* allele_blob; uint32_t* allele_len; int32_t* ci; int32_t* num_spanning;
  int32_t* classification; int32_t* read_rank; uint32_t* n_spanning_reads;
  uint8_t* flipped;
  int32_t* gt_size;
  const uint8_t* genotyper;
  uint8_t* skip_b;
  int32_t finish_clears_need;
  RepairBufs rp;
  const uint32_t *sel_read, *sel_start, *sel_len, *n_sel;
};
struct GtFlankArgs : GtArgs {
  const int16_t* hp_tag;
  uint8_t* flank_done;
};
struct SnvArgs : GtFlankArgs {
  const int32_t *start_offset, *end_offset;
  const int32_t* mismatch_offsets; const uint64_t* mismatch_off;
  uint8_t* snv_read;
  double ln_match, ln_mis, ln2;
  int32_t tag_route;
};
template <bool FLANK, bool SNV = false> using GtArgsOf = std::conditional_t<SNV, SnvArgs, std::conditional_t<FLANK, GtFlankArgs, GtArgs>>;

template <int MAXR, bool FLANK> struct FlankShared {};
template <int MAXR> struct FlankShared<MAXR, true> {
  uint16_t f_uidx[MAXR];
  uint16_t f_cnt[2][MAXR];
  uint32_t f_med[2][2];
};
template <int MAXR, bool SNV> struct SnvShared {};
template <int MAXR> struct SnvShared<MAXR, true> {
  int32_t v_so[MAXR], v_eo[MAXR];
  union {
    int32_t offs[SNV_OFFS_PER_READ * MAXR];
    struct { uint64_t obs[MAXR], val[MAXR]; } p;
  } v;
  int32_t v_snv[SNV_MAX_SNVS], v_tmp[SNV_MAX_SNVS];
  uint64_t v_hap[SNV_MAX_HAPS];
  double v_ll[SNV_MAX_HAPS * (SNV_MAX_HAPS + 1) / 2];
  uint8_t v_tie[MAXR];
  int32_t v_reg[2];
};
template <int MAXR, int SEG, bool FLANK = false, bool SNV = false>
struct GtShared : FlankShared<MAXR, FLANK>, SnvShared<MAXR, SNV> {
  uint32_t r_s[MAXR], r_len[MAXR];
  uint64_t r_off[MAXR];
  uint32_t s_read[MAXR], s_start[MAXR], s_len[MAXR];
  uint16_t s_loff[MAXR];
  uint16_t u_rep[MAXR], u_cnt[MAXR];
  uint32_t ulen[MAXR], ucnt[MAXR];
  int8_t cls[MAXR];
  int n, n_sizes, bail, fits;
  int res_n_gt, res_flip, res_rep[2], res_ci[4], res_hap[2];
  Reserved rsv;
  uint32_t ref_off;
  alignas(16) uint8_t bytes[SEG];
};

__device__ __forceinline__ uint32_t adiff_u(uint32_t a, uint32_t b) { return a > b ? a - b : b - a; }

__device__ __forceinline__ int cmp_lds(const uint8_t* a, uint32_t na, const uint8_t* b, uint32_t nb) {
  const int lane = threadIdx.x & 63;
  const uint32_t m = na < nb ? na : nb;
  const uint32_t* A = reinterpret_cast<const uint32_t*>(a); const uint32_t* B = reinterpret_cast<const uint32_t*>(b);
  const uint32_t nw = (m + 3u) >> 2;
  for (uint32_t base = 0; base < nw; base += 64) {
    const uint32_t w = base + (uint32_t)lane;
    uint32_t x = 0, y = 0;
    if (w < nw) {
      x = A[w]; y = B[w];
      if (w == nw - 1 && (m & 3u)) { const uint32_t mask = (1u << (8 * (m & 3u))) - 1u; x &= mask; y &= mask; }
    }
    const unsigned long long ne = __ballot(x != y);
    if (ne) {
      const int f = __ffsll((long long)ne) - 1;
      const uint32_t xf = (uint32_t)__builtin_amdgcn_readlane((int)x, f), yf = (uint32_t)__builtin_amdgcn_readlane((int)y, f);
      return __builtin_bswap32(xf) < __builtin_bswap32(yf) ? -1 : 1;
// ... 329 lines not shown
    const int i = base + lane;
    uint64_t obs = 0, val = 0;
    if (i < n) {
      const uint64_t r = r0 + sh.s_read[i];
      const int32_t* m = a.mismatch_offsets + a.mismatch_off[r];
      const int nm = (int)(a.mismatch_off[r + 1] - a.mismatch_off[r]);
      const int32_t s = sh.v_so[i], e = sh.v_eo[i];
      for (int k = 0; k < ns; ++k) {
        const int32_t o = sh.v_snv[k];
        if (o < s || o > e) continue;
        obs |= 1ull << k;
        int lo = 0, hi = nm;
        while (lo < hi) { const int mid = (lo + hi) >> 1; if (m[mid] < o) lo = mid + 1; else hi = mid; }
        if (lo < nm && m[lo] == o) val |= 1ull << k;
      }
      sh.v.p.obs[i] = obs; sh.v.p.val[i] = val;
    }
    full += __popcll(__ballot(i < n && obs == all));
  }
  __syncthreads();
  if ((double)full / (double)n < 0.40) return nosplit();
  int nh = 0;
  for (int base = 0; base < n; base += 64) {
    const int i = base + lane;
    bool first = i < n && sh.v.p.obs[i] == all;
    if (first) { const uint64_t v = sh.v.p.val[i]; for (int j = 0; j < i; ++j) first = first && !(sh.v.p.obs[j] == all && sh.v.p.val[j] == v); }
    if (i < n) sh.v_tie[i] = first ? 1 : 0;
    nh += __popcll(__ballot(first));
  }
  __syncthreads();
  if (nh * (nh + 1) / 2 <= 1) return nosplit();
  if (nh > SNV_MAX_HAPS) return handed(0);
  for (int i = lane; i < n; i += 64) {
    if (!sh.v_tie[i]) continue;
    const uint64_t key = __brevll(sh.v.p.val[i]);
    int r = 0;
    for (int j = 0; j < n; ++j) r += sh.v_tie[j] && __brevll(sh.v.p.val[j]) < key;
    sh.v_hap[r] = sh.v.p.val[i];
  }
  __syncthreads();
  const int nc = nh * (nh + 1) / 2;
  for (int c = lane; c < nc; c += 64) {
    int ha = 0, hb = 0;
    { int p = 0; for (int x = 0; x < nh; ++x) for (int y = x; y < nh; ++y, ++p) if (p == c) { ha = x; hb = y; } }
    sh.v_ll[c] = snv_candidate_ll(a, n, ns, sh.v_hap[ha], sh.v_hap[hb], [&](int i, uint64_t& obs, uint64_t& val) { obs = sh.v.p.obs[i]; val = sh.v.p.val[i]; });
  }
  __syncthreads();
  double M = sh.v_ll[0]; int win = 0;
  for (int c = 1; c < nc; ++c) if (sh.v_ll[c] >= M) { M = sh.v_ll[c]; win = c; }
  const double delta = 0x1p-30 * (1.0 + fabs(M));
  bool decided = true;
  for (int c = 0; c < nc; ++c) if (c != win && sh.v_ll[c] >= M - delta) decided = false;
  if (!decided) return handed(FL_UNDECIDED);
  int wa = 0, wb = 0;
  { int p = 0; for (int x = 0; x < nh; ++x) for (int y = x; y < nh; ++y, ++p) if (p == win) { wa = x; wb = y; } }
  if (wa == wb) return nosplit();
  const uint64_t top1 = sh.v_hap[wa], top2 = sh.v_hap[wb];
  __syncthreads();
  int ties = 0, cnt[2] = {0, 0}, hap[2] = {0, 0};
  for (int base = 0; base < n; base += 64) {
    const int i = base + lane;
    int d1 = 0, d2 = 0;
    if (i < n) { const uint64_t obs = sh.v.p.obs[i], val = sh.v.p.val[i]; d1 = __popcll(obs & ~(val ^ top1)); d2 = __popcll(obs & ~(val ^ top2)); }
    const bool tie = i < n && d1 == d2;
    const unsigned long long tb = __ballot(tie);
    const int k = ties + __popcll(tb & ((1ull << lane) - 1ull));
    const int g = tie ? (k & 1) : (d1 < d2 ? 0 : 1);
    if (i < n) { sh.cls[i] = (int8_t)g; sh.v_tie[i] = tie ? 1 : 0; }
    const int here = n - base < 64 ? n - base : 64;
    const int ones = __popcll(__ballot(i < n && g == 1)), m1 = __popcll(__ballot(i < n && (g == 1 || tie))), m0 = __popcll(__ballot(i < n && (g == 0 || tie)));
    hap[1] += ones; hap[0] += here - ones; cnt[0] += m0; cnt[1] += m1;
    ties += __popcll(tb);
  }
  __syncthreads();
  if constexpr (END::SIZE) {
    if (!flank_tail<SnvMembers>(sh, a, l, n, nu, lane, fits, refn, refo, cnt, hap, (uint8_t)FL_SNV)) return nosplit();
    if (sh.bail == 2)
      for (int i = lane; i < n; i += 64)
        a.snv_read[r0 + i] = (uint8_t)((sh.cls[i] ? SR_ASSIGN : 0) | (SnvMembers::in(sh, i, 0) ? SR_IN0 : 0) | (SnvMembers::in(sh, i, 1) ? SR_IN1 : 0));
    return true;
  } else return END::split(sh, a, l, lane, cnt, hap);
}

template <int MAXR, int SEG, bool PRESEL = false, bool FLANK = false, bool SNV = false>
__global__ void __launch_bounds__(64) locus_genotype_kernel(const GtArgsOf<FLANK, SNV> a) {
  static_assert(FLANK || !SNV, "the SNV forms are FLANK forms: they share the tail of the route and its LDS");
  __shared__ GtShared<MAXR, SEG, FLANK, SNV> sh;
  const int64_t l = blockIdx.x;
  if (l >= a.n_loci) return;
  const int lane = threadIdx.x;
  const uint64_t r0 = a.locus_read_begin[l], r1 = a.locus_read_begin[l + 1];
  const int nr = (int)(r1 - r0);
  if (lane == 0) {
    sh.n = 0; sh.bail = 0; sh.fits = 1; sh.res_n_gt = 0;
    if (a.gt_size) a.gt_size[2 * l] = a.gt_size[2 * l + 1] = 0;
    if (a.skip_b) a.skip_b[l] = 1;
    a.need_host[l] = 0; a.n_alleles[l] = 0; a.n_spanning_reads[l] = 0; a.flipped[l] = 0;
    a.allele_len[2 * l] = a.allele_len[2 * l + 1] = 0; a.num_spanning[2 * l] = a.num_spanning[2 * l + 1] = 0;
    if constexpr (FLANK) a.flank_done[l] = 0;
  }
  const bool cluster = a.genotyper && a.genotyper[l] == 1;
  if (a.ploidy[l] == 0 || nr == 0 || nr > MAXR || cluster) {
    for (int i = lane; i < nr; i += 64) { a.classification[r0 + i] = -1; a.read_rank[r0 + i] = -1; }
    if (lane == 0 && (nr > MAXR || cluster) && a.ploidy[l] != 0 && nr != 0) a.need_host[l] = 1;
    return;
  }
  gt_selected<MAXR, PRESEL>(sh, a, l, r0, nr, lane);
  const uint32_t refn = a.tr_len[l];
  const uint64_t refo = a.tr_off[l];
  int n = sh.n;
  if (n > 0) {
    if (lane == 0) {
      uint32_t o = 0;
      const int nn = sh.n;
      for (int i = 0; i < nn; ++i) { sh.s_loff[i] = (uint16_t)o; o += (sh.s_len[i] + 3u) & ~3u; if (o > (uint32_t)SEG) { sh.fits = 0; break; } }
      sh.ref_off = o;
      if (o + ((refn + 3u) & ~3u) > (uint32_t)SEG) sh.fits = 0;
    }
    __syncthreads();
    n = sh.n;
    if (sh.fits) {
      const int grp = lane >> 4, sub = lane & 15;
      for (int i = grp; i < n; i += 4) copy16(sh.bytes + sh.s_loff[i], a.reads + sh.r_off[sh.s_read[i]] + sh.s_start[i], sh.s_len[i], sub);
      if (grp == 0) copy16(sh.bytes + sh.ref_off, a.tr_blob + refo, refn, sub);
    }
    __syncthreads();
  }
  const bool fits = sh.fits != 0;
  auto seg_glob = [&](int i) { return a.reads + sh.r_off[sh.s_read[i]] + sh.s_start[i]; };
  auto cmp_seg = [&](int i, int j) {
    return fits ? cmp_lds(sh.bytes + sh.s_loff[i], sh.s_len[i], sh.bytes + sh.s_loff[j], sh.s_len[j]) : cmp_bytes(seg_glob(i), sh.s_len[i], seg_glob(j), sh.s_len[j]);
  };
  if (n > 0 && !sh.bail) {
    if (lane == 0) {
      int u = 0;
      for (int i = 0; i < n; ++i) {
        const uint32_t v = sh.s_len[i];
        int p = 0;
        while (p < u && sh.ulen[p] < v) ++p;
        if (p < u && sh.ulen[p] == v) { sh.ucnt[p] += 1; continue; }
        for (int q = u; q > p; --q) { sh.ulen[q] = sh.ulen[q - 1]; sh.ucnt[q] = sh.ucnt[q - 1]; }
        sh.ulen[p] = v; sh.ucnt[p] = 1; ++u;
      }
      sh.n_sizes = u;
    }
    __syncthreads();
    const int u = sh.n_sizes;
    const int ploidy = a.ploidy[l] == 1 ? 1 : 2;
    double best_pen = 0.0; int best_p = 0x7FFFFFFF; bool have = false;
    if (ploidy == 2) {
      int p = 0;
      for (int si = 0; si < u; ++si)
        for (int li = si; li < u; ++li, ++p) {
          if ((p & 63) != lane) continue;
          const uint32_t sa = sh.ulen[si], la = sh.ulen[li];
          const double max_frac = adiff_u(sa, la) <= 100 ? 0.25 : 0.05;
          double pen = 0.0;
          for (int i = 0; i < u; ++i) {
            const uint32_t st = sh.ulen[i] != sa ? 10 + 2 * adiff_u(sa, sh.ulen[i]) : 0, lt = sh.ulen[i] != la ? 10 + 2 * adiff_u(la, sh.ulen[i]) : 0;
            const double term = (double)(st < lt ? st : lt) + max_frac * (double)(st > lt ? st : lt);
            pen += term * (double)sh.ucnt[i];
          }
          if (!have || pen < best_pen) { have = true; best_pen = pen; best_p = p; }
        }
    } else {
      for (int c = lane; c < u; c += 64) {
        double pen = 0.0;
        for (int i = 0; i < u; ++i) {
          const double term = sh.ulen[i] != sh.ulen[c] ? 10.0 + 2.0 * (double)adiff_u(sh.ulen[c], sh.ulen[i]) : 0.0;
          pen += term * (double)sh.ucnt[i];
        }
        if (!have || pen < best_pen) { have = true; best_pen = pen; best_p = c; }
      }
    }
    for (int o = 32; o > 0; o >>= 1) {
      const double op = __shfl_xor(best_pen, o); const int oi = __shfl_xor(best_p, o); const int oh = __shfl_xor((int)have, o);
      if (oh && (!have || op < best_pen || (op == best_pen && oi < best_p))) { have = true; best_pen = op; best_p = oi; }
    }
    {
      uint32_t size[2] = {0, 0}, civ[4] = {0, 0, 0, 0};
      int n_gt;
      if (ploidy == 2) {
        int si = 0, li = 0, p = 0;
        for (int x = 0; x < u; ++x) for (int y = x; y < u; ++y, ++p) if (p == best_p) { si = x; li = y; }
        const uint32_t bs = sh.ulen[si], bl = sh.ulen[li];
        uint32_t short_size = bs < bl ? bs : bl, long_size = bs > bl ? bs : bl;
        if (short_size != long_size && u >= 2) {
          uint64_t coverage = 0; int top = 0;
          for (int i = 0; i < u; ++i) { coverage += sh.ucnt[i]; if (sh.ucnt[i] > sh.ucnt[top]) top = i; }
          const double top_frac = (double)sh.ucnt[top] / (double)coverage;
          const uint32_t range = sh.ulen[u - 1] - sh.ulen[0];
          if (top_frac > 0.60 && range <= 6) short_size = long_size = sh.ulen[top];
        }
        n_gt = 2; size[0] = short_size; size[1] = long_size;
        civ[0] = civ[1] = short_size; civ[2] = civ[3] = long_size;
        for (int i = 0; i < u; ++i) {
          const uint32_t s = sh.ulen[i];
          if (adiff_u(s, short_size) <= adiff_u(s, long_size)) { civ[0] = civ[0] < s ? civ[0] : s; civ[1] = civ[1] > s ? civ[1] : s; }
          else { civ[2] = civ[2] < s ? civ[2] : s; civ[3] = civ[3] > s ? civ[3] : s; }
        }
      } else {
        n_gt = 1; size[0] = sh.ulen[best_p];
        civ[0] = sh.ulen[0]; civ[1] = sh.ulen[u - 1];
      }
      int nu = 0;
      for (int i = 0; i < n; ++i) {
        int lo = 0, hi = nu, eq = -1;
        while (lo < hi) {
          const int mid = (lo + hi) >> 1;
          const int r = sh.u_rep[mid];
          const int c = cmp_seg(i, r);
          if (c == 0) { eq = mid; break; }
          if (c < 0) hi = mid; else lo = mid + 1;
        }
        if (eq >= 0) { if (lane == 0) { sh.u_cnt[eq] += 1; if constexpr (FLANK) sh.f_uidx[i] = sh.u_rep[eq]; } continue; }
        if (lane == 0) {
          for (int q = nu; q > lo; --q) { sh.u_rep[q] = sh.u_rep[q - 1]; sh.u_cnt[q] = sh.u_cnt[q - 1]; }
          sh.u_rep[lo] = (uint16_t)i; sh.u_cnt[lo] = 1;
          if constexpr (FLANK) sh.f_uidx[i] = (uint16_t)i;
        }
        ++nu;
      }
      bool by_tags = false;
      if constexpr (SNV) {
        if (n_gt == 2 && adiff_u(size[0], size[1]) <= 10) {
          int cnt[2];
          if (a.hp_tag && flank_assign(sh, a.hp_tag, r0, n, lane, cnt)) by_tags = a.tag_route && flank_tail<TagMembers>(sh, a, l, n, nu, lane, fits, refn, refo, cnt, cnt, (uint8_t)0);
          else by_tags = snv_route<MAXR>(sh, a, l, r0, n, nu, lane, fits, refn, refo);
        }
      } else if constexpr (FLANK) {
        if (a.hp_tag && n_gt == 2 && adiff_u(size[0], size[1]) <= 10) by_tags = flank_route(sh, a, l, r0, n, nu, lane, fits, refn, refo);
      }
      auto ulen_of = [&](int q) { return sh.s_len[sh.u_rep[q]]; };
      auto closest = [&](uint32_t target) { uint32_t c = ulen_of(0); for (int q = 0; q < nu; ++q) if (adiff_u(c, target) > adiff_u(ulen_of(q), target)) c = ulen_of(q); return c; };
      auto most_frequent = [&](uint32_t len) { int best = -1; for (int q = 0; q < nu; ++q) if (ulen_of(q) == len && (best < 0 || sh.u_cnt[q] >= sh.u_cnt[best])) best = q; return best; };
      int pick[2] = {most_frequent(closest(size[0])), -1};
      int n_pick = 1;
      if (n_gt != 1 && size[0] != size[1]) { pick[1] = most_frequent(closest(size[1])); n_pick = 2; }
      bool majority = true, lacks[2] = {false, false};
      auto in_group = [&](int q, int al) {
        if (n_gt == 1) return true;
        const uint32_t d1 = adiff_u(ulen_of(q), size[0]), d2 = adiff_u(ulen_of(q), size[1]);
        return al == 0 ? d1 <= d2 : d2 < d1;
      };
      for (int al = 0; al < n_pick; ++al) {
        uint64_t coverage = 0, ref_count = 0;
        for (int q = 0; q < nu; ++q) {
          if (!in_group(q, al)) continue;
          coverage += sh.u_cnt[q];
          if (q == pick[al]) ref_count = sh.u_cnt[q];
        }
        if (!(2 * ref_count >= coverage)) { majority = false; lacks[al] = true; }
      }
      if (by_tags) {}
      else if (!majority) {
        const RepairBufs& rp = a.rp;
        bool can = rp.counts != nullptr;
        uint32_t nm[2] = {0, 0}; unsigned long long mbytes[2] = {0, 0};
        if (can)
          for (int al = 0; al < n_pick; ++al) {
            if (!lacks[al]) continue;
            if (ulen_of(pick[al]) > rp.max_seg) can = false;
            for (int q = 0; q < nu; ++q) {
              if (!in_group(q, al)) continue;
              if (ulen_of(q) > rp.max_seg) can = false;
              nm[al] += 1; mbytes[al] += ulen_of(q);
            }
          }
        GroupNeeds nd[2] = {};
        if (can) {
#pragma unroll
          for (int al = 0; al < 2; ++al) if (lacks[al]) nd[al] = group_needs(ulen_of(pick[al]), nm[al], mbytes[al], rp.vote_lds_pos);
          if (lane == 0) repair_reserve(rp, l, a.n_loci, nm[0] + nm[1], (uint32_t)lacks[0] + (uint32_t)lacks[1], nd, sh.rsv);
          __syncthreads();
          can = sh.rsv.ok != 0;
        }
        if (!can) sh.bail = 1;
        else {
          Reserved at = sh.rsv;
          auto seg_of = [&](int q) { const int r = sh.u_rep[q]; return Seg{sh.r_off[sh.s_read[r]] + sh.s_start[r], sh.s_len[r]}; };
          RepairPend pd;
          pd.n_gt = n_gt; pd.n_pick = n_pick; pd.size[0] = size[0]; pd.size[1] = size[1];
          for (int k = 0; k < 4; ++k) pd.civ[k] = (int32_t)civ[k];
          pd.rep[0] = pd.rep[1] = -1; pd.grp[0] = pd.grp[1] = -1;
#pragma unroll
          for (int al = 0; al < 2; ++al) {
            if (al >= n_pick) break;
            pd.rep[al] = sh.u_rep[pick[al]];
            if (lacks[al]) pd.grp[al] = (int32_t)queue_group<64>(rp.groups, rp.jobs, at, seg_of(pick[al]), nm[al], nd[al], nu, [&, al](int q) { return in_group(q, al); }, seg_of);
          }
          if (lane == 0) rp.pend[l] = pd;
          sh.bail = 2;
        }
      }
      else {
        int rep[2]; uint32_t aln[2];
        for (int al = 0; al < n_pick; ++al) { rep[al] = sh.u_rep[pick[al]]; aln[al] = sh.s_len[rep[al]]; }
        int n_al = n_pick;
        if (ploidy == 2 && n_al == 1) { rep[1] = rep[0]; aln[1] = aln[0]; n_al = 2; }
        int by_hap[2] = {0, 0}, tie = 1;
        for (int i = 0; i < n; ++i) {
          int cc = 0;
          if (n_al == 2) {
            const uint32_t d1 = adiff_u(sh.s_len[i], aln[0]), d2 = adiff_u(sh.s_len[i], aln[1]);
            if (d1 < d2) cc = 0; else if (d1 > d2) cc = 1; else { tie = (tie + 1) % 2; cc = tie; }
          }
          sh.cls[i] = (int8_t)cc; by_hap[cc] += 1;
        }
        auto eq_ref = [&](int al) {
          return fits ? cmp_lds(sh.bytes + sh.s_loff[rep[al]], aln[al], sh.bytes + sh.ref_off, refn) == 0 : cmp_bytes(seg_glob(rep[al]), aln[al], a.tr_blob + refo, refn) == 0;
        };
        int order[2] = {0, 1}; int flip = 0;
        if (n_gt != 1 && !eq_ref(0) && eq_ref(1)) { order[0] = 1; order[1] = 0; flip = 1; }
        for (int oi = 0; oi < n_gt; ++oi)
          if (aln[order[oi]] > a.allele_cap[l]) sh.bail = 1;
        sh.res_n_gt = n_gt; sh.res_flip = flip;
        for (int oi = 0; oi < n_gt; ++oi) {
          const int al = order[oi];
          sh.res_rep[oi] = rep[al]; sh.res_ci[2 * oi] = (int)civ[2 * al]; sh.res_ci[2 * oi + 1] = (int)civ[2 * al + 1]; sh.res_hap[oi] = by_hap[al];
        }
      }
    }
    __syncthreads();
  }
  const bool done = n > 0 && !sh.bail;
  for (int i = lane; i < nr; i += 64) { a.classification[r0 + i] = -1; a.read_rank[r0 + i] = -1; }
  if (n > 0 && sh.bail) { if (lane == 0) a.need_host[l] = (uint8_t)(sh.bail == 2 ? 2 : 1); return; }
  if (!done) return;
  __syncthreads();
  const int n_gt = sh.res_n_gt;
  for (int oi = 0; oi < n_gt; ++oi) {
    const int rep = sh.res_rep[oi];
    const uint32_t len = sh.s_len[rep];
    const uint8_t* src = fits ? sh.bytes + sh.s_loff[rep] : seg_glob(rep);
    uint8_t* dst = a.allele_blob + a.allele_off[2 * l + oi];
    for (uint32_t b = lane; b < len; b += 64) dst[b] = src[b];
    if (lane == 0) {
      a.allele_len[2 * l + oi] = len;
      a.ci[4 * l + 2 * oi] = sh.res_ci[2 * oi]; a.ci[4 * l + 2 * oi + 1] = sh.res_ci[2 * oi + 1];
      a.num_spanning[2 * l + oi] = sh.res_hap[oi];
      if (a.gt_size) a.gt_size[2 * l + oi] = (int32_t)len;
    }
  }
  for (int i = lane; i < n; i += 64) {
    a.classification[r0 + sh.s_read[i]] = sh.res_flip ? 1 - sh.cls[i] : sh.cls[i];
    a.read_rank[r0 + sh.s_read[i]] = i;
  }
  if (lane == 0) { a.n_alleles[l] = n_gt; a.n_spanning_reads[l] = (uint32_t)n; a.flipped[l] = (uint8_t)sh.res_flip; }
}

template <int MAXR>
struct FinShared {
  uint32_t r_s[MAXR], r_len[MAXR]; uint64_t r_off[MAXR];
  uint32_t s_read[MAXR], s_start[MAXR], s_len[MAXR];
  int8_t cls[MAXR];
  int n;
};
__device__ __forceinline__ bool wave_equal(const uint8_t* __restrict__ p, uint32_t n, const uint8_t* __restrict__ q, uint32_t m) {
  if (n != m) return false;
  bool diff = false;
  for (uint32_t i = threadIdx.x & 63; i < n; i += 64) diff = diff || p[i] != q[i];
  return __ballot(diff) == 0ull;
}
template <class SH>
__device__ __forceinline__ void flank_finish(SH& sh, const GtFlankArgs& a, const FinishArgs& f, const RepairPend& pd, int64_t l, uint64_t r0, int n, int lane,
                                             const uint8_t* __restrict__ snv = nullptr) {
  const RepairBufs& rp = a.rp;
  int cnt[2] = {0, 0};
  const uint8_t mark = snv ? (uint8_t)FL_SNV : (uint8_t)0;
  bool fail;
  if (snv) {
    for (int base = 0; base < n; base += 64) {
      const int i = base + lane;
      const int g = i < n ? snv[r0 + i] & SR_ASSIGN : 0;
      if (i < n) sh.cls[i] = (int8_t)g;
      const int ones = __popcll(__ballot(i < n && g == 1));
      cnt[1] += ones; cnt[0] += (n - base < 64 ? n - base : 64) - ones;
    }
    __syncthreads();
    fail = n == 0;
  } else fail = n == 0 || !flank_assign(sh, a.hp_tag, r0, n, lane, cnt);
  const uint8_t* ap[2] = {nullptr, nullptr}; uint32_t aln[2] = {0, 0};
  auto seg_of = [&](int i) { return Seg{sh.r_off[sh.s_read[i]] + sh.s_start[i], sh.s_len[i]}; };
  for (int g = 0; g < 2 && !fail; ++g) fail = !repaired_allele(pd, g, f, rp, a.reads, seg_of, ap[g], aln[g]);
  const int sw = aln[0] > aln[1] ? 1 : 0;
  int order[2] = {sw, 1 - sw}, flip = 0;
  if (!fail) {
    const uint8_t* ref = a.tr_blob + a.tr_off[l]; const uint32_t refn = a.tr_len[l];
    if (!wave_equal(ap[order[0]], aln[order[0]], ref, refn) && wave_equal(ap[order[1]], aln[order[1]], ref, refn)) { order[0] = 1 - sw; order[1] = sw; flip = 1; }
    if (aln[0] > a.allele_cap[l] || aln[1] > a.allele_cap[l]) fail = true;
  }
  if (fail) { if (lane == 0) { a.need_host[l] = 1; a.flank_done[l] = FL_HANDED | mark; } return; }
  for (int oi = 0; oi < 2; ++oi) {
    const int g = order[oi];
    uint8_t* dst = a.allele_blob + a.allele_off[2 * l + oi];
    for (uint32_t b = lane; b < aln[g]; b += 64) dst[b] = ap[g][b];
    if (lane == 0) {
      a.allele_len[2 * l + oi] = aln[g];
      a.ci[4 * l + 2 * oi] = pd.civ[2 * g]; a.ci[4 * l + 2 * oi + 1] = pd.civ[2 * g + 1];
      a.num_spanning[2 * l + oi] = cnt[g];
      if (a.gt_size) a.gt_size[2 * l + oi] = (int32_t)aln[g];
    }
  }
  for (int i = lane; i < n; i += 64) {
    a.classification[r0 + sh.s_read[i]] = sh.cls[i] == order[0] ? 0 : 1;
    a.read_rank[r0 + sh.s_read[i]] = i;
  }
  if (lane == 0) {
    a.n_alleles[l] = 2; a.n_spanning_reads[l] = (uint32_t)n; a.flipped[l] = (uint8_t)flip; a.skip_b[l] = 0; if (a.finish_clears_need) a.need_host[l] = 0;
    a.flank_done[l] = FL_DONE | FL_REPAIRED | mark;
  }
}
template <int MAXR, bool PRESEL = false, bool FLANK = false, bool SNV = false>
__global__ void __launch_bounds__(64) repair_finish_kernel(const GtArgsOf<FLANK, SNV> a, const FinishArgs f) {
  __shared__ FinShared<MAXR> sh;
  const RepairBufs& rp = a.rp;
  if (blockIdx.x >= rp.counts[RC_LOCI]) return;
  const int64_t l = rp.loci[blockIdx.x];
  const int lane = threadIdx.x;
  const uint64_t r0 = a.locus_read_begin[l];
  const int nr = (int)(a.locus_read_begin[l + 1] - r0);
  if (nr > MAXR) return;
  if (lane == 0) sh.n = 0;
  gt_selected<MAXR, PRESEL>(sh, a, l, r0, nr, lane);
  const int n = sh.n;
  const RepairPend pd = rp.pend[l];
  if constexpr (FLANK) {
    if constexpr (SNV) {
      if (pd.n_pick & RP_SNV) { flank_finish(sh, a, f, pd, l, r0, n, lane, a.snv_read); return; }
    }
    if (pd.n_pick & RP_FLANK) { flank_finish(sh, a, f, pd, l, r0, n, lane); return; }
// ... 47 lines not shown
```

### trgt_amd/csrc/repair_queue.hpp

```cpp
#pragma once
#include "common.hpp"
#include "wfa_host.hpp"

namespace trgt {
namespace gt {

struct RGroup {
  uint32_t job_first, n_members, bb_len, out_cap;
  uint64_t bb_off, out_off, scratch_off;
};
struct RepairPend {
  int32_t n_gt, n_pick; uint32_t size[2]; int32_t civ[4]; int32_t rep[2] ; int32_t grp[2] ;
};
enum { RC_GROUPS = 0, RC_JOBS = 1, RC_LOCI = 2, RC_FAILED = 3, RC_CIGAR = 4 , RC_OUT = 6 , RC_SCRATCH = 8 , RC_REFUSED = 10 , RC_WORDS = 16 };
struct RepairBufs {
  uint32_t* counts;
  RGroup* groups; JobDev* jobs; uint32_t* loci; RepairPend* pend;
  uint32_t cap_groups, cap_jobs, max_seg, vote_lds_pos;
  uint64_t cap_cigar, cap_out, cap_scratch;
};
struct FinishArgs { const uint8_t* vote_out; const uint32_t* vote_len; };

struct GroupNeeds { unsigned long long cig, out_need, scr_need; uint32_t out_cap; };
__device__ __forceinline__ GroupNeeds group_needs(uint32_t bb, uint32_t nm, unsigned long long mbytes, uint32_t vote_lds_pos) {
  GroupNeeds nd;
  nd.cig = (unsigned long long)nm * ((unsigned long long)bb + 1) + mbytes;
  nd.out_cap = (uint32_t)(bb + mbytes + 16);
  nd.out_need = ((unsigned long long)nd.out_cap + 15ull) & ~15ull;
  nd.scr_need = (bb + 1 <= vote_lds_pos + 1 ? 0ull : 3ull * ((unsigned long long)bb + 1)) + 3ull * nm;
  return nd;
}

struct Reserved { int ok; uint32_t g0, j0; unsigned long long c0, o0, s0; };
static_assert(sizeof(Reserved) == 40, "the six words every kernel's LDS held for it");

__device__ __forceinline__ bool reserve_arenas(uint32_t* cigar, uint32_t* out, uint32_t* scratch, uint64_t cap_cigar, uint64_t cap_out, uint64_t cap_scratch,
                                               const GroupNeeds (&nd)[2], Reserved& r) {
  auto take = [](uint32_t* counter, unsigned long long need, unsigned long long cap, unsigned long long& base) {
    base = atomicAdd(reinterpret_cast<unsigned long long*>(counter), need);
    return base + need <= cap;
  };
  r.c0 = r.o0 = r.s0 = 0;
  r.ok = take(cigar, nd[0].cig + nd[1].cig, cap_cigar, r.c0) && take(out, nd[0].out_need + nd[1].out_need, cap_out, r.o0) &&
         take(scratch, nd[0].scr_need + nd[1].scr_need, cap_scratch, r.s0);
  return r.ok != 0;
}

__device__ __forceinline__ void repair_reserve(const RepairBufs& rp, int64_t l, int64_t n_loci, uint32_t n_jobs, uint32_t n_groups, const GroupNeeds (&nd)[2], Reserved& r) {
  if (!reserve_arenas(rp.counts + RC_CIGAR, rp.counts + RC_OUT, rp.counts + RC_SCRATCH, rp.cap_cigar, rp.cap_out, rp.cap_scratch, nd, r)) { atomicAdd(rp.counts + RC_FAILED, 1u); return; }
  r.j0 = atomicAdd(rp.counts + RC_JOBS, n_jobs);
  r.g0 = atomicAdd(rp.counts + RC_GROUPS, n_groups);
  if (r.j0 + n_jobs > rp.cap_jobs || r.g0 + 2 > rp.cap_groups) r.ok = 0;
  else { const uint32_t slot = atomicAdd(rp.counts + RC_LOCI, 1u); if (slot < (uint32_t)n_loci) rp.loci[slot] = (uint32_t)l; else r.ok = 0; }
}

struct Seg { unsigned long long off; uint32_t len; };
__device__ __forceinline__ void put_group(RGroup* groups, const Reserved& at, Seg bb, uint32_t nm, const GroupNeeds& nd) {
  RGroup G;
  G.job_first = at.j0; G.n_members = nm; G.bb_len = bb.len; G.out_cap = nd.out_cap;
  G.bb_off = bb.off; G.out_off = at.o0; G.scratch_off = at.s0;
  groups[at.g0] = G;
}
__device__ __forceinline__ void put_job(JobDev* jobs, uint32_t j, Seg bb, Seg member, unsigned long long cigar_off) {
  JobDev jd;
  jd.pat_off = bb.off; jd.pat_len = bb.len;
  jd.txt_off = member.off; jd.txt_len = member.len;
  jd.cigar_off = cigar_off; jd.ops_off = 0; jd.out_index = j; jd.pad = 0;
  jobs[j] = jd;
}
template <int W, class IsMember, class SegOf>
__device__ __forceinline__ uint32_t queue_group(RGroup* groups, JobDev* jobs, Reserved& at, Seg bb, uint32_t nm, const GroupNeeds& nd, int n, IsMember is_member, SegOf seg) {
  const uint32_t g = at.g0;
  if (threadIdx.x == 0) put_group(groups, at, bb, nm, nd);
  uint32_t k = 0;
  for (int i = 0; i < n; ++i) {
    if (!is_member(i)) continue;
    if ((k & (uint32_t)(W - 1)) == threadIdx.x) put_job(jobs, at.j0 + k, bb, seg(i), at.c0);
    at.c0 += (unsigned long long)bb.len + seg(i).len + 1;
    ++k;
  }
  at.j0 += nm; at.o0 += nd.out_need; at.s0 += nd.scr_need; ++at.g0;
  return g;
}

template <class SegOf>
__device__ __forceinline__ bool repaired_allele(const RepairPend& pd, int al, const FinishArgs& f, const RepairBufs& rp, const uint8_t* reads, SegOf seg, const uint8_t*& p, uint32_t& len) {
  if (pd.grp[al] >= 0) {
    const uint32_t voted = f.vote_len[pd.grp[al]];
    if (voted == 0xFFFFFFFFu) return false;
    p = f.vote_out + rp.groups[pd.grp[al]].out_off; len = voted;
  } else { const Seg s = seg(pd.rep[al]); p = reads + s.off; len = s.len; }
  return true;
}

}
}
```

Before: 5.140 million loci/s.

## Parallelize size genotyper stages across wave lanes and use wave-level block prefix scans

Replaces the serial single-thread prefix sums in the span and allele prefix kernels with a wave-shuffle block scan. In the device size genotyper, the serial per-locus loops for layout, read staging, length runs, duplicate-read detection (via hashing), candidate picking, classification and output writeback become wave-cooperative ballot and shuffle versions. The old serial paths are kept behind dev flags, and optional profiling counters are added. This targets long serial per-locus loops on a single lane, at the cost of more complex code and a hash-then-verify equality check.

```diff
diff --git a/trgt_amd/csrc/common.hpp b/trgt_amd/csrc/common.hpp
--- a/trgt_amd/csrc/common.hpp
+++ b/trgt_amd/csrc/common.hpp
@@ -47,6 +47,8 @@
   bool no_early = false;
   bool stage_lock = false;
   bool host_hmm_lists = false;
+  bool gt_serial = false;
+  bool gt_weak_hash = false;
   bool debug = false;
   bool hmm_resolve_one_wg = false;
   bool wfa_no_wave_variant = false;
@@ -318,6 +320,33 @@
   return TRGT_OK;
 }
 
+static __device__ __forceinline__ void block_prefix_u32(const uint32_t* __restrict__ v, uint64_t* __restrict__ off, uint64_t n) {
+  typedef unsigned long long u64;
+  __shared__ u64 wave_total[16];
+  const uint32_t lane = threadIdx.x & 63u, wave = threadIdx.x >> 6;
+  const uint64_t per = ((n + 63) / 64 + 15) / 16 * 64;
+  const uint64_t b = (uint64_t)wave * per < n ? (uint64_t)wave * per : n, e = b + per < n ? b + per : n;
+  u64 s = 0;
+  for (uint64_t i = b + lane; i < e; i += 64) s += v[i];
+  for (int o = 32; o > 0; o >>= 1) s += __shfl_xor(s, o);
+  if (lane == 0) wave_total[wave] = s;
+  __syncthreads();
+  u64 run = 0;
+  for (uint32_t w = 0; w < wave; ++w) run += wave_total[w];
+  if (threadIdx.x == 1023) off[n] = run + s;
+  for (uint64_t base = b; base < e; base += 256) {
+    u64 x[4], inc[4];
+#pragma unroll
+    for (int k = 0; k < 4; ++k) { const uint64_t i = base + 64 * k + lane; x[k] = i < e ? v[i] : 0; inc[k] = x[k]; }
+    for (int o = 1; o < 64; o <<= 1) {
+#pragma unroll
+      for (int k = 0; k < 4; ++k) { const u64 y = __shfl_up(inc[k], o); if (lane >= (uint32_t)o) inc[k] += y; }
+    }
+#pragma unroll
+    for (int k = 0; k < 4; ++k) { const uint64_t i = base + 64 * k + lane; if (i < e) off[i] = run + inc[k] - x[k]; run += __shfl(inc[k], 63); }
+  }
+}
+
 constexpr size_t ZERO_ARENA_BYTES = 2u << 20;
 static __global__ void zero_arena_kernel(uint4* __restrict__ p, size_t n16) {
   for (size_t i = (size_t)blockIdx.x * blockDim.x + threadIdx.x; i < n16; i += (size_t)gridDim.x * blockDim.x) p[i] = make_uint4(0u, 0u, 0u, 0u);
diff --git a/trgt_amd/csrc/ctx.hip b/trgt_amd/csrc/ctx.hip
--- a/trgt_amd/csrc/ctx.hip
+++ b/trgt_amd/csrc/ctx.hip
@@ -75,6 +75,7 @@
     (void)num; (void)flag;
     k.flank_threads = DEV_NUM("TRGT_FLANK_THREADS", k.flank_threads); k.heavy_threads = DEV_NUM("TRGT_HEAVY_THREADS", 0); k.heavy_band = std::max(0, std::min(num("TRGT_HEAVY_BAND", k.heavy_band), 256));
     k.win_threads = DEV_NUM("TRGT_WIN_THREADS", k.win_threads); { const int bt = DEV_NUM("TRGT_BAND_THREADS", k.band_threads); k.band_threads = bt == 128 || bt == 256 ? bt : 64; } k.win_segments = DEV_NUM("TRGT_WIN_SEGMENTS", k.win_segments); k.win_lds = DEV_FLAG("TRGT_WIN_LDS"); k.band_lds = DEV_FLAG("TRGT_BAND_LDS");
+    k.gt_serial = DEV_FLAG("TRGT_GT_SERIAL"); k.gt_weak_hash = DEV_FLAG("TRGT_GT_WEAK_HASH");
     k.grid_per_cu = DEV_NUM("TRGT_WFA_GRID_PER_CU", 0); k.filter_per_cu = DEV_NUM("TRGT_FILTER_PER_CU", 0);
     k.one_launch = DEV_FLAG("TRGT_WFA_ONE_LAUNCH"); k.no_spec = DEV_FLAG("TRGT_WFA_NO_SPEC"); k.no_window = flag("TRGT_WFA_NO_WINDOW"); k.no_hamming = flag("TRGT_NO_HAMMING"); k.no_indel_shortcut = flag("TRGT_NO_INDEL_SHORTCUT"); k.no_heavy_window = DEV_FLAG("TRGT_NO_HEAVY_WINDOW"); k.no_sibling_rule = DEV_FLAG("TRGT_NO_SIBLING_RULE"); k.no_settled_sibling_rule = DEV_FLAG("TRGT_NO_SETTLED_SIBLING_RULE"); k.no_lcs_rule = DEV_FLAG("TRGT_NO_LCS_RULE"); { const char* e = TRGT_DEV_ENV("TRGT_EARLY_ADAPTIVE"); if (e && *e) k.early_adaptive = std::strcmp(e, "0") != 0; }
     k.no_filter = flag("TRGT_WFA_NO_FILTER"); k.one_stream = DEV_FLAG("TRGT_FLANK_ONE_STREAM"); k.host_genotyper = flag("TRGT_HOST_GENOTYPER"); k.host_hmm_lists = DEV_FLAG("TRGT_HOST_HMM_LISTS"); k.no_early = flag("TRGT_WFA_NO_EARLY"); k.stage_lock = flag("TRGT_STAGE_LOCK"); k.no_long_filter = flag("TRGT_NO_LONG_FILTER"); k.no_long_window = DEV_FLAG("TRGT_NO_LONG_WINDOW"); k.filter_force = DEV_NUM("TRGT_FILTER_FORCE", 0); k.filter_one_launch = DEV_FLAG("TRGT_FILTER_ONE_LAUNCH"); k.filter_serial = DEV_FLAG("TRGT_FILTER_SERIAL"); k.filter_side = DEV_FLAG("TRGT_FILTER_SIDE"); k.wfa_no_stage = DEV_FLAG("TRGT_WFA_NO_STAGE"); k.wfa_no_wave_variant = DEV_FLAG("TRGT_WFA_NO_WAVE_VARIANT"); k.hmm_resolve_one_wg = DEV_FLAG("TRGT_HMM_RESOLVE_ONE_WG"); k.debug = flag("TRGT_WFA_DEBUG");
diff --git a/trgt_amd/csrc/hmm.hip b/trgt_amd/csrc/hmm.hip
--- a/trgt_amd/csrc/hmm.hip
+++ b/trgt_amd/csrc/hmm.hip
@@ -1438,17 +1438,7 @@
 }
 
 __global__ void __launch_bounds__(1024) hmm_span_prefix_kernel(const uint32_t* __restrict__ n_spans, uint64_t* __restrict__ off, uint64_t n) {
-  __shared__ uint64_t part[1024];
-  const uint32_t t = threadIdx.x;
-  const uint64_t per = (n + 1023) / 1024, b = t * per < n ? t * per : n, e = b + per < n ? b + per : n;
-  uint64_t sum = 0;
-  for (uint64_t i = b; i < e; ++i) sum += n_spans[i];
-  part[t] = sum;
-  __syncthreads();
-  if (t == 0) { uint64_t run = 0; for (int i = 0; i < 1024; ++i) { const uint64_t v = part[i]; part[i] = run; run += v; } off[n] = run; }
-  __syncthreads();
-  uint64_t run = part[t];
-  for (uint64_t i = b; i < e; ++i) { off[i] = run; run += n_spans[i]; }
+  block_prefix_u32(n_spans, off, n);
 }
 
 
diff --git a/trgt_amd/csrc/locus.hip b/trgt_amd/csrc/locus.hip
--- a/trgt_amd/csrc/locus.hip
+++ b/trgt_amd/csrc/locus.hip
@@ -443,20 +443,11 @@
 
 struct CountCopy { const uint32_t* src1; uint32_t* dst1; uint32_t n1; const uint32_t* src2; uint32_t* dst2; uint32_t n2; const uint32_t* src3; uint32_t* dst3; uint32_t n3; };
 __global__ void __launch_bounds__(1024) allele_prefix_kernel(const uint32_t* __restrict__ len, uint64_t* __restrict__ off, int64_t n, const CountCopy cc) {
-  __shared__ uint64_t part[1024];
   const int t = threadIdx.x;
   if ((uint32_t)t < cc.n1) cc.dst1[t] = cc.src1 ? __hip_atomic_load(cc.src1 + t, __ATOMIC_RELAXED, __HIP_MEMORY_SCOPE_AGENT) : 0u;
   if ((uint32_t)t < cc.n2) cc.dst2[t] = cc.src2 ? __hip_atomic_load(cc.src2 + t, __ATOMIC_RELAXED, __HIP_MEMORY_SCOPE_AGENT) : 0u;
   if ((uint32_t)t < cc.n3) cc.dst3[t] = cc.src3 ? __hip_atomic_load(cc.src3 + t, __ATOMIC_RELAXED, __HIP_MEMORY_SCOPE_AGENT) : 0u;
-  const int64_t per = (n + 1023) / 1024, b = t * per, e = b + per < n ? b + per : n;
-  uint64_t sum = 0;
-  for (int64_t i = b; i < e; ++i) sum += len[i];
-  part[t] = sum;
-  __syncthreads();
-  if (t == 0) { uint64_t run = 0; for (int i = 0; i < 1024; ++i) { const uint64_t v = part[i]; part[i] = run; run += v; } off[n] = run; }
-  __syncthreads();
-  uint64_t run = part[t];
-  for (int64_t i = b; i < e; ++i) { off[i] = run; run += len[i]; }
+  block_prefix_u32(len, off, (uint64_t)n);
 }
 __global__ void allele_pack_kernel(const uint8_t* __restrict__ blob, const uint64_t* __restrict__ src_off, const uint32_t* __restrict__ len,
                                    const uint64_t* __restrict__ dst_off, uint8_t* __restrict__ packed, int64_t n) {
@@ -695,6 +686,7 @@
   enum class GtForm { PLAIN, FLANK, SNV };
   GtForm gt_form() const { return fits[FR_SIZE_SNV] ? GtForm::SNV : fits[FR_SIZE_TAG] ? GtForm::FLANK : GtForm::PLAIN; }
   void launch_genotype_kernels(), launch_finish_kernels(const gt::FinishArgs& fa);
+  int gt_prof_readback();
   void tally_route(FlankRoute r, const std::vector<uint32_t>* list, uint8_t snv, const uint8_t* fdone, const uint8_t* need);
   gt::GtFlankArgs flank_args() const { gt::GtFlankArgs fa; static_cast<gt::GtArgs&>(fa) = ga; fa.hp_tag = g.hp; fa.flank_done = (uint8_t*)slab.d(o_fdone); return fa; }
   gt::SnvArgs snv_args() const {
@@ -1123,9 +1115,26 @@
       break;
   }
 }
+int LocusCall::gt_prof_readback() {
+#ifdef TRGT_GT_PROF
+  if (!c->knobs.debug) return TRGT_OK;
+  unsigned long long h[gt::GTP_WORDS], z[gt::GTP_WORDS] = {0};
+  TRGT_HIP_TRY(c, trgt::stream_wait(c, c->stream));
+  TRGT_HIP_TRY(c, hipMemcpyFromSymbol(h, HIP_SYMBOL(gt::g_gt_prof), sizeof h));
+  TRGT_HIP_TRY(c, hipMemcpyToSymbol(HIP_SYMBOL(gt::g_gt_prof), z, sizeof h));
+  double tot = 1e-9;
+  for (int i = 0; i <= gt::GTP_OUT; ++i) tot += (double)h[i];
+  fprintf(stderr, "[gt prof] %lld loci, %s reads | front %.1f%% staging %.1f%% lengths %.1f%% candidates %.1f%% sequences %.1f%% routes %.1f%% picks %.1f%% classification %.1f%% outputs %.1f%% | kcycles per locus %.1f\n",
+          (long long)nl, small_gt ? "<= 64" : "<= 256", 100 * h[gt::GTP_FRONT] / tot, 100 * h[gt::GTP_STAGE] / tot, 100 * h[gt::GTP_LENS] / tot, 100 * h[gt::GTP_CAND] / tot, 100 * h[gt::GTP_SEQ] / tot,
+          100 * h[gt::GTP_ROUTE] / tot, 100 * h[gt::GTP_PICK] / tot, 100 * h[gt::GTP_CLASS] / tot, 100 * h[gt::GTP_OUT] / tot, tot / 1e3 / (double)std::max<int64_t>(1, nl));
+#endif
+  return TRGT_OK;
+}
 int LocusCall::size_genotyper() {
   if (!dev_gt) return TRGT_OK;
+  ga.finish_clears_need = (c->knobs.gt_serial ? gt::GT_DEV_SERIAL : 0) | (c->knobs.gt_weak_hash ? gt::GT_DEV_WEAK_HASH : 0);
   launch_genotype_kernels();
+  if (int prc = gt_prof_readback()) return prc;
   ran[FR_SIZE_TAG] = fits[FR_SIZE_TAG]; ran[FR_SIZE_SNV] = fits[FR_SIZE_SNV];
   TRGT_HIP_TRY(c, hipGetLastError());
   tl_mark(c, "genotyper launched");
@@ -1169,16 +1178,17 @@
   LR.pat_base = d_reads; LR.txt_base = d_reads;
   LR.max_plen = rp.max_seg; LR.max_tlen = rp.max_seg; LR.max_sum = 2 * (int64_t)rp.max_seg;
   LR.cigar = (uint32_t*)rb.cig; LR.cigar_len = (uint32_t*)rb.clen; LR.buffer_set = 2; LR.ws_budget = 512ull << 20; LR.refused = rp.counts + gt::RC_REFUSED;
-  auto dbg_sync = [&](const char* what) -> int {
+  auto dbg_sync = [&](const char* what, bool size_gt = false) -> int {
     if (!c->knobs.debug) return TRGT_OK;
     const hipError_t e = trgt::stream_wait(c, c->stream);
     uint32_t h[gt::RC_WORDS]; std::memset(h, 0, sizeof h);
     if (e == hipSuccess) (void)hipMemcpy(h, rp.counts, sizeof h, hipMemcpyDeviceToHost);
     fprintf(stderr, "[repair] %s: %s (groups %u jobs %u loci %u failed %u cigar words %llu)\n", what, hipGetErrorString(e), h[gt::RC_GROUPS], h[gt::RC_JOBS], h[gt::RC_LOCI], h[gt::RC_FAILED],
             (unsigned long long)h[gt::RC_CIGAR] | ((unsigned long long)h[gt::RC_CIGAR + 1] << 32));
+    if (size_gt) fprintf(stderr, "[size gt] of %lld loci: unsorted %u, not staged %u, hash collision %u\n", (long long)nl, h[gt::RC_GT_UNSORTED], h[gt::RC_GT_NOFIT], h[gt::RC_GT_COLLISION]);
     return e == hipSuccess ? TRGT_OK : fail(c, TRGT_ERR_HIP, "%s failed: %s", what, hipGetErrorString(e));
   };
-  if ((rc = dbg_sync("genotyper"))) return rc;
+  if ((rc = dbg_sync("genotyper", true))) return rc;
   if (uint32_t* trace_host = repair_trace_buf()) { std::memset(trace_host, 0, 4096); hipLaunchKernelGGL(repair_trace_kernel, dim3(1), dim3(64), 0, c->stream, rp, trace_host); }
   static const bool repair_check = TRGT_DEV_ENV("TRGT_REPAIR_CHECK") != nullptr;
   if (repair_check) {
diff --git a/trgt_amd/csrc/locus_gt.hpp b/trgt_amd/csrc/locus_gt.hpp
--- a/trgt_amd/csrc/locus_gt.hpp
+++ b/trgt_amd/csrc/locus_gt.hpp
@@ -18,6 +18,7 @@
 constexpr int SNV_OFFS_PER_READ = 8;
 enum { SR_ASSIGN = 1, SR_IN0 = 2, SR_IN1 = 4 };
 
+enum { GT_DEV_SERIAL = 2, GT_DEV_WEAK_HASH = 4 };
 struct GtArgs {
   const uint8_t* reads; const uint64_t* read_off; const uint32_t* read_len; const uint64_t* locus_read_begin;
   const int32_t* span_start; const int32_t* span_end;
@@ -513,6 +514,148 @@
   } else return END::split(sh, a, l, lane, cnt, hap);
 }
 
+__device__ __forceinline__ uint32_t wave_sum_u(uint32_t v) { for (int o = 32; o > 0; o >>= 1) v += (uint32_t)__shfl_xor((int)v, o); return v; }
+__device__ __forceinline__ uint32_t wave_incl_sum_u(uint32_t v, int lane) {
+  for (int o = 1; o < 64; o <<= 1) { const uint32_t w = (uint32_t)__shfl_up((int)v, o); if (lane >= o) v += w; }
+  return v;
+}
+__device__ __forceinline__ void gt_tally(const RepairBufs& rp, int word, int lane) { if (lane == 0 && rp.counts) atomicAdd(rp.counts + word, 1u); }
+
+template <int MAXR, int SEG, class SH>
+__device__ __forceinline__ void gt_layout(SH& sh, int n, uint32_t refn, int lane) {
+  uint32_t carry = 0; bool over = false;
+  for (int base = 0; base < n; base += 64) {
+    const int i = base + lane;
+    const uint32_t v = i < n ? (sh.s_len[i] + 3u) & ~3u : 0u;
+    const uint32_t inc = wave_incl_sum_u(v, lane);
+    if (i < n) sh.s_loff[i] = (uint16_t)(carry + inc - v);
+    over = over || __ballot(i < n && carry + inc > (uint32_t)SEG) != 0ull;
+    carry += (uint32_t)__builtin_amdgcn_readlane((int)inc, 63);
+  }
+  if (lane == 0) { sh.ref_off = carry; if (over || carry + ((refn + 3u) & ~3u) > (uint32_t)SEG) sh.fits = 0; }
+}
+
+template <int K, class SH>
+__device__ __forceinline__ void gt_stage(SH& sh, const GtArgs& a, int n, uint32_t refn, uint64_t refo, int lane) {
+  const int grp = lane >> 4, sub = lane & 15;
+  for (int j0 = grp * K; j0 <= n; j0 += 4 * K) {
+    const uint8_t* src[K]; uint8_t* dst[K]; uint32_t len[K];
+#pragma unroll
+    for (int k = 0; k < K; ++k) {
+      const int j = j0 + k;
+      src[k] = a.tr_blob + refo; dst[k] = sh.bytes + sh.ref_off; len[k] = j == n ? refn : 0u;
+      if (j < n) { src[k] = a.reads + sh.r_off[sh.s_read[j]] + sh.s_start[j]; dst[k] = sh.bytes + sh.s_loff[j]; len[k] = sh.s_len[j]; }
+    }
+    uint4 v[K]; uint8_t tl[K];
+#pragma unroll
+    for (int k = 0; k < K; ++k) {
+      const uint32_t full = len[k] >> 4, tb = full * 16 + (uint32_t)sub;
+      if ((uint32_t)sub < full) __builtin_memcpy(&v[k], src[k] + 16 * sub, 16);
+      if (tb < len[k]) tl[k] = src[k][tb];
+    }
+#pragma unroll
+    for (int k = 0; k < K; ++k) {
+      const uint32_t full = len[k] >> 4, tb = full * 16 + (uint32_t)sub;
+      if ((uint32_t)sub < full) { uint32_t* d = reinterpret_cast<uint32_t*>(dst[k]) + 4 * sub; d[0] = v[k].x; d[1] = v[k].y; d[2] = v[k].z; d[3] = v[k].w; }
+      if (tb < len[k]) dst[k][tb] = tl[k];
+    }
+#pragma unroll
+    for (int k = 0; k < K; ++k)
+      for (uint32_t w = 16 + (uint32_t)sub; w < (len[k] >> 4); w += 16) {
+        uint4 x; __builtin_memcpy(&x, src[k] + 16 * w, 16);
+        uint32_t* d = reinterpret_cast<uint32_t*>(dst[k]) + 4 * w;
+        d[0] = x.x; d[1] = x.y; d[2] = x.z; d[3] = x.w;
+      }
+  }
+}
+
+template <int MAXR, class SH>
+__device__ __forceinline__ bool gt_len_runs(SH& sh, int n, int lane) {
+  int u = 0; bool sorted = true;
+  for (int base = 0; base < n; base += 64) {
+    const int i = base + lane;
+    const uint32_t cur = i < n ? sh.s_len[i] : 0u, prev = i > 0 && i < n ? sh.s_len[i - 1] : 0u;
+    sorted = sorted && __ballot(i > 0 && i < n && prev > cur) == 0ull;
+    const bool begin = i < n && (i == 0 || prev != cur);
+    const unsigned long long bb = __ballot(begin);
+    if (begin) { const int s = u + __popcll(bb & ((1ull << lane) - 1ull)); sh.ulen[s] = cur; sh.ucnt[s] = (uint32_t)i; }
+    u += __popcll(bb);
+  }
+  if (!sorted) return false;
+  __syncthreads();
+  uint32_t at[MAXR / 64], next[MAXR / 64];
+#pragma unroll
+  for (int t = 0; t < MAXR / 64; ++t) { const int s = lane + 64 * t; if (s < u) { at[t] = sh.ucnt[s]; next[t] = s + 1 < u ? sh.ucnt[s + 1] : (uint32_t)n; } }
+  __syncthreads();
+#pragma unroll
+  for (int t = 0; t < MAXR / 64; ++t) { const int s = lane + 64 * t; if (s < u) sh.ucnt[s] = next[t] - at[t]; }
+  if (lane == 0) sh.n_sizes = u;
+  return true;
+}
+
+template <int R, class SH>
+__device__ __forceinline__ bool gt_equal_reads(SH& sh, int n, int lane, bool weak, int (&fr)[R]) {
+  uint32_t ln[R], h1[R], h2[R];
+#pragma unroll
+  for (int t = 0; t < R; ++t) {
+    const int i = lane + 64 * t;
+    ln[t] = 0; h1[t] = 0x811C9DC5u; h2[t] = 0x9E3779B9u; fr[t] = -1;
+    if (i >= n) continue;
+    ln[t] = sh.s_len[i];
+    if (weak) continue;
+    const uint32_t* W = reinterpret_cast<const uint32_t*>(sh.bytes + sh.s_loff[i]);
+    const uint32_t nw = (ln[t] + 3u) >> 2, tail = (ln[t] & 3u) ? (1u << (8 * (ln[t] & 3u))) - 1u : 0xFFFFFFFFu;
+    for (uint32_t w = 0; w < nw; w += 4) {
+      uint32_t x[4];
+#pragma unroll
+      for (uint32_t k = 0; k < 4; ++k) { x[k] = w + k < nw ? W[w + k] : 0u; if (w + k == nw - 1) x[k] &= tail; }
+#pragma unroll
+      for (uint32_t k = 0; k < 4; ++k) {
+        h1[t] = (h1[t] ^ x[k]) * 0x9E3779B1u; h1[t] = (h1[t] << 13) | (h1[t] >> 19);
+        h2[t] = (h2[t] + x[k]) * 0x85EBCA6Bu; h2[t] ^= h2[t] >> 15;
+      }
+    }
+  }
+#pragma unroll
+  for (int tj = 0; tj < R; ++tj)
+    for (int jl = 0; jl < 64 && 64 * tj + jl < n; ++jl) {
+      const uint32_t lj = (uint32_t)__builtin_amdgcn_readlane((int)ln[tj], jl), a1 = (uint32_t)__builtin_amdgcn_readlane((int)h1[tj], jl),
+                     a2 = (uint32_t)__builtin_amdgcn_readlane((int)h2[tj], jl);
+#pragma unroll
+      for (int t = 0; t < R; ++t)
+        if (fr[t] < 0 && lane + 64 * t < n && ln[t] == lj && h1[t] == a1 && h2[t] == a2) fr[t] = 64 * tj + jl;
+    }
+  bool differ = false;
+#pragma unroll
+  for (int t = 0; t < R; ++t) {
+    const int i = lane + 64 * t;
+    if (i >= n || fr[t] == i) continue;
+    const uint32_t* A = reinterpret_cast<const uint32_t*>(sh.bytes + sh.s_loff[i]);
+    const uint32_t* B = reinterpret_cast<const uint32_t*>(sh.bytes + sh.s_loff[fr[t]]);
+    const uint32_t nw = (ln[t] + 3u) >> 2, tail = (ln[t] & 3u) ? (1u << (8 * (ln[t] & 3u))) - 1u : 0xFFFFFFFFu;
+    for (uint32_t w = 0; w < nw; w += 4) {
+#pragma unroll
+      for (uint32_t k = 0; k < 4; ++k) {
+        if (w + k >= nw) break;
+        uint32_t x = A[w + k] ^ B[w + k];
+        if (w + k == nw - 1) x &= tail;
+        differ = differ || x != 0u;
+      }
+    }
+  }
+  return __ballot(differ) == 0ull;
+}
+
+enum { GTP_FRONT = 0, GTP_STAGE, GTP_LENS, GTP_CAND, GTP_SEQ, GTP_ROUTE, GTP_PICK, GTP_CLASS, GTP_OUT, GTP_WORDS = 16 };
+#ifdef TRGT_GT_PROF
+__device__ unsigned long long g_gt_prof[GTP_WORDS];
+#define GTP_DECL unsigned long long gtp_t = clock64()
+#define GTP_MARK(i) do { const unsigned long long n_ = clock64(); if (threadIdx.x == 0) atomicAdd(&g_gt_prof[i], n_ - gtp_t); gtp_t = n_; } while (0)
+#else
+#define GTP_DECL
+#define GTP_MARK(i)
+#endif
+
 template <int MAXR, int SEG, bool PRESEL = false, bool FLANK = false, bool SNV = false>
 __global__ void __launch_bounds__(64) locus_genotype_kernel(const GtArgsOf<FLANK, SNV> a) {
   static_assert(FLANK || !SNV, "the SNV forms are FLANK forms: they share the tail of the route and its LDS");
@@ -520,8 +663,14 @@
   const int64_t l = blockIdx.x;
   if (l >= a.n_loci) return;
   const int lane = threadIdx.x;
+  constexpr int R = MAXR / 64;
+  const bool serial = (a.finish_clears_need & GT_DEV_SERIAL) != 0, weak_hash = (a.finish_clears_need & GT_DEV_WEAK_HASH) != 0;
   const uint64_t r0 = a.locus_read_begin[l], r1 = a.locus_read_begin[l + 1];
   const int nr = (int)(r1 - r0);
+  const uint8_t ploidy_l = a.ploidy[l];
+  const uint32_t refn = a.tr_len[l], allele_cap_l = a.allele_cap[l];
+  const uint64_t refo = a.tr_off[l], allele_at[2] = {a.allele_off[2 * l], a.allele_off[2 * l + 1]};
+  GTP_DECL;
   if (lane == 0) {
     sh.n = 0; sh.bail = 0; sh.fits = 1; sh.res_n_gt = 0;
     if (a.gt_size) a.gt_size[2 * l] = a.gt_size[2 * l + 1] = 0;
@@ -531,39 +680,43 @@
     if constexpr (FLANK) a.flank_done[l] = 0;
   }
   const bool cluster = a.genotyper && a.genotyper[l] == 1;
-  if (a.ploidy[l] == 0 || nr == 0 || nr > MAXR || cluster) {
+  if (ploidy_l == 0 || nr == 0 || nr > MAXR || cluster) {
     for (int i = lane; i < nr; i += 64) { a.classification[r0 + i] = -1; a.read_rank[r0 + i] = -1; }
-    if (lane == 0 && (nr > MAXR || cluster) && a.ploidy[l] != 0 && nr != 0) a.need_host[l] = 1;
+    if (lane == 0 && (nr > MAXR || cluster) && ploidy_l != 0 && nr != 0) a.need_host[l] = 1;
     return;
   }
   gt_selected<MAXR, PRESEL>(sh, a, l, r0, nr, lane);
-  const uint32_t refn = a.tr_len[l];
-  const uint64_t refo = a.tr_off[l];
   int n = sh.n;
+  GTP_MARK(GTP_FRONT);
   if (n > 0) {
-    if (lane == 0) {
+    if (!serial) gt_layout<MAXR, SEG>(sh, n, refn, lane);
+    else if (lane == 0) {
       uint32_t o = 0;
-      const int nn = sh.n;
-      for (int i = 0; i < nn; ++i) { sh.s_loff[i] = (uint16_t)o; o += (sh.s_len[i] + 3u) & ~3u; if (o > (uint32_t)SEG) { sh.fits = 0; break; } }
+      for (int i = 0; i < n; ++i) { sh.s_loff[i] = (uint16_t)o; o += (sh.s_len[i] + 3u) & ~3u; if (o > (uint32_t)SEG) { sh.fits = 0; break; } }
       sh.ref_off = o;
       if (o + ((refn + 3u) & ~3u) > (uint32_t)SEG) sh.fits = 0;
     }
     __syncthreads();
-    n = sh.n;
     if (sh.fits) {
-      const int grp = lane >> 4, sub = lane & 15;
-      for (int i = grp; i < n; i += 4) copy16(sh.bytes + sh.s_loff[i], a.reads + sh.r_off[sh.s_read[i]] + sh.s_start[i], sh.s_len[i], sub);
-      if (grp == 0) copy16(sh.bytes + sh.ref_off, a.tr_blob + refo, refn, sub);
+      if (!serial) gt_stage<4>(sh, a, n, refn, refo, lane);
+      else {
+        const int grp = lane >> 4, sub = lane & 15;
+        for (int i = grp; i < n; i += 4) copy16(sh.bytes + sh.s_loff[i], a.reads + sh.r_off[sh.s_read[i]] + sh.s_start[i], sh.s_len[i], sub);
+        if (grp == 0) copy16(sh.bytes + sh.ref_off, a.tr_blob + refo, refn, sub);
+      }
     }
     __syncthreads();
   }
   const bool fits = sh.fits != 0;
-  auto seg_glob = [&](int i) { return a.reads + sh.r_off[sh.s_read[i]] + sh.s_start[i]; };
+  GTP_MARK(GTP_STAGE);
+  auto seg_glob =[&](int i) { return a.reads + sh.r_off[sh.s_read[i]] + sh.s_start[i]; };
   auto cmp_seg = [&](int i, int j) {
     return fits ? cmp_lds(sh.bytes + sh.s_loff[i], sh.s_len[i], sh.bytes + sh.s_loff[j], sh.s_len[j]) : cmp_bytes(seg_glob(i), sh.s_len[i], seg_glob(j), sh.s_len[j]);
   };
   if (n > 0 && !sh.bail) {
-    if (lane == 0) {
+    const bool runs = !serial && gt_len_runs<MAXR>(sh, n, lane);
+    if (!runs && !serial) gt_tally(a.rp, RC_GT_UNSORTED, lane);
+    if (!runs && lane == 0) {
       int u = 0;
       for (int i = 0; i < n; ++i) {
         const uint32_t v = sh.s_len[i];
@@ -577,7 +730,8 @@
     }
     __syncthreads();
     const int u = sh.n_sizes;
-    const int ploidy = a.ploidy[l] == 1 ? 1 : 2;
+    GTP_MARK(GTP_LENS);
+    const int ploidy = ploidy_l == 1 ? 1 : 2;
     double best_pen = 0.0; int best_p = 0x7FFFFFFF; bool have = false;
     if (ploidy == 2) {
       int p = 0;
@@ -608,6 +762,7 @@
       const double op = __shfl_xor(best_pen, o); const int oi = __shfl_xor(best_p, o); const int oh = __shfl_xor((int)have, o);
       if (oh && (!have || op < best_pen || (op == best_pen && oi < best_p))) { have = true; best_pen = op; best_p = oi; }
     }
+    GTP_MARK(GTP_CAND);
     {
       uint32_t size[2] = {0, 0}, civ[4] = {0, 0, 0, 0};
       int n_gt;
@@ -634,24 +789,46 @@
         n_gt = 1; size[0] = sh.ulen[best_p];
         civ[0] = sh.ulen[0]; civ[1] = sh.ulen[u - 1];
       }
+      GTP_MARK(GTP_CAND);
+      int fr[R];
+      bool grouped = fits && !serial;
+      if (grouped) { grouped = gt_equal_reads<R>(sh, n, lane, weak_hash, fr); if (!grouped) gt_tally(a.rp, RC_GT_COLLISION, lane); }
+      else if (!serial) gt_tally(a.rp, RC_GT_NOFIT, lane);
+      unsigned long long first[R];
+#pragma unroll
+      for (int t = 0; t < R; ++t) {
+        const int i = lane + 64 * t;
+        if (!grouped) fr[t] = i < n ? i : -1;
+        first[t] = __ballot(i < n && fr[t] == i);
+        if constexpr (FLANK) { if (i < n) sh.f_uidx[i] = (uint16_t)fr[t]; }
+      }
+      __syncthreads();
       int nu = 0;
-      for (int i = 0; i < n; ++i) {
-        int lo = 0, hi = nu, eq = -1;
-        while (lo < hi) {
-          const int mid = (lo + hi) >> 1;
-          const int r = sh.u_rep[mid];
-          const int c = cmp_seg(i, r);
-          if (c == 0) { eq = mid; break; }
-          if (c < 0) hi = mid; else lo = mid + 1;
-        }
-        if (eq >= 0) { if (lane == 0) { sh.u_cnt[eq] += 1; if constexpr (FLANK) sh.f_uidx[i] = sh.u_rep[eq]; } continue; }
-        if (lane == 0) {
-          for (int q = nu; q > lo; --q) { sh.u_rep[q] = sh.u_rep[q - 1]; sh.u_cnt[q] = sh.u_cnt[q - 1]; }
-          sh.u_rep[lo] = (uint16_t)i; sh.u_cnt[lo] = 1;
-          if constexpr (FLANK) sh.f_uidx[i] = (uint16_t)i;
-        }
-        ++nu;
-      }
+#pragma unroll
+      for (int t = 0; t < R; ++t) {
+        for (unsigned long long m = first[t]; m; m &= m - 1ull) {
+          const int i = 64 * t + __ffsll((long long)m) - 1;
+          int mult = 0;
+#pragma unroll
+          for (int tt = 0; tt < R; ++tt) mult += __popcll(__ballot(fr[tt] == i));
+          int lo = 0, hi = nu, eq = -1;
+          while (lo < hi) {
+            const int mid = (lo + hi) >> 1;
+            const int r = sh.u_rep[mid];
+            const int c = cmp_seg(i, r);
+            if (c == 0) { eq = mid; break; }
+            if (c < 0) hi = mid; else lo = mid + 1;
+          }
+          if (eq >= 0) { if (lane == 0) { sh.u_cnt[eq] += (uint16_t)mult; if constexpr (FLANK) sh.f_uidx[i] = sh.u_rep[eq]; } continue; }
+          if (lane == 0) {
+            for (int q = nu; q > lo; --q) { sh.u_rep[q] = sh.u_rep[q - 1]; sh.u_cnt[q] = sh.u_cnt[q - 1]; }
+            sh.u_rep[lo] = (uint16_t)i; sh.u_cnt[lo] = (uint16_t)mult;
+          }
+          ++nu;
+        }
+      }
+      __syncthreads();
+      GTP_MARK(GTP_SEQ);
       bool by_tags = false;
       if constexpr (SNV) {
         if (n_gt == 2 && adiff_u(size[0], size[1]) <= 10) {
@@ -663,26 +840,68 @@
         if (a.hp_tag && n_gt == 2 && adiff_u(size[0], size[1]) <= 10) by_tags = flank_route(sh, a, l, r0, n, nu, lane, fits, refn, refo);
       }
       auto ulen_of = [&](int q) { return sh.s_len[sh.u_rep[q]]; };
-      auto closest = [&](uint32_t target) { uint32_t c = ulen_of(0); for (int q = 0; q < nu; ++q) if (adiff_u(c, target) > adiff_u(ulen_of(q), target)) c = ulen_of(q); return c; };
-      auto most_frequent = [&](uint32_t len) { int best = -1; for (int q = 0; q < nu; ++q) if (ulen_of(q) == len && (best < 0 || sh.u_cnt[q] >= sh.u_cnt[best])) best = q; return best; };
+      GTP_MARK(GTP_ROUTE);
+      uint32_t ql[R], qc[R];
+#pragma unroll
+      for (int t = 0; t < R; ++t) { const int q = lane + 64 * t; ql[t] = q < nu ? ulen_of(q) : 0u; qc[t] = q < nu ? sh.u_cnt[q] : 0u; }
+      auto len_in_group = [&](uint32_t len, int al) {
+        if (n_gt == 1) return true;
+        const uint32_t d1 = adiff_u(len, size[0]), d2 = adiff_u(len, size[1]);
+        return al == 0 ? d1 <= d2 : d2 < d1;
+      };
+      auto in_group = [&](int q, int al) { return len_in_group(ulen_of(q), al); };
+      auto closest = [&](uint32_t target) {
+        if (serial) { uint32_t c = ulen_of(0); for (int q = 0; q < nu; ++q) if (adiff_u(c, target) > adiff_u(ulen_of(q), target)) c = ulen_of(q); return c; }
+        uint32_t d[R], best = 0xFFFFFFFFu;
+#pragma unroll
+        for (int t = 0; t < R; ++t) { d[t] = lane + 64 * t < nu ? adiff_u(ql[t], target) : 0xFFFFFFFFu; best = d[t] < best ? d[t] : best; }
+        best = wave_min_u(best);
+        uint32_t c = 0;
+#pragma unroll
+        for (int t = R - 1; t >= 0; --t) {
+          const unsigned long long bal = __ballot(lane + 64 * t < nu && d[t] == best);
+          if (bal) c = (uint32_t)__builtin_amdgcn_readlane((int)ql[t], __ffsll((long long)bal) - 1);
+        }
+        return c;
+      };
+      auto most_frequent = [&](uint32_t len) {
+        if (serial) { int best = -1; for (int q = 0; q < nu; ++q) if (ulen_of(q) == len && (best < 0 || sh.u_cnt[q] >= sh.u_cnt[best])) best = q; return best; }
+        uint32_t mx = 0;
+#pragma unroll
+        for (int t = 0; t < R; ++t) if (lane + 64 * t < nu && ql[t] == len && qc[t] > mx) mx = qc[t];
+        mx = wave_max_u(mx);
+        int best = -1;
+#pragma unroll
+        for (int t = 0; t < R; ++t) {
+          const unsigned long long bal = __ballot(lane + 64 * t < nu && ql[t] == len && qc[t] == mx);
+          if (bal) best = 64 * t + 63 - __clzll((long long)bal);
+        }
+        return best;
+      };
       int pick[2] = {most_frequent(closest(size[0])), -1};
       int n_pick = 1;
       if (n_gt != 1 && size[0] != size[1]) { pick[1] = most_frequent(closest(size[1])); n_pick = 2; }
       bool majority = true, lacks[2] = {false, false};
-      auto in_group = [&](int q, int al) {
-        if (n_gt == 1) return true;
-        const uint32_t d1 = adiff_u(ulen_of(q), size[0]), d2 = adiff_u(ulen_of(q), size[1]);
-        return al == 0 ? d1 <= d2 : d2 < d1;
-      };
       for (int al = 0; al < n_pick; ++al) {
         uint64_t coverage = 0, ref_count = 0;
-        for (int q = 0; q < nu; ++q) {
-          if (!in_group(q, al)) continue;
-          coverage += sh.u_cnt[q];
-          if (q == pick[al]) ref_count = sh.u_cnt[q];
+        if (serial) {
+          for (int q = 0; q < nu; ++q) {
+            if (!in_group(q, al)) continue;
+            coverage += sh.u_cnt[q];
+            if (q == pick[al]) ref_count = sh.u_cnt[q];
+          }
+        } else {
+          uint32_t cov = 0, ref = 0;
+#pragma unroll
+          for (int t = 0; t < R; ++t) {
+            const int q = lane + 64 * t;
+            if (q < nu && len_in_group(ql[t], al)) { cov += qc[t]; if (q == pick[al]) ref = qc[t]; }
+          }
+          coverage = wave_sum_u(cov); ref_count = wave_sum_u(ref);
         }
         if (!(2 * ref_count >= coverage)) { majority = false; lacks[al] = true; }
       }
+      GTP_MARK(GTP_PICK);
       if (by_tags) {}
       else if (!majority) {
         const RepairBufs& rp = a.rp;
@@ -729,14 +948,33 @@
         for (int al = 0; al < n_pick; ++al) { rep[al] = sh.u_rep[pick[al]]; aln[al] = sh.s_len[rep[al]]; }
         int n_al = n_pick;
         if (ploidy == 2 && n_al == 1) { rep[1] = rep[0]; aln[1] = aln[0]; n_al = 2; }
-        int by_hap[2] = {0, 0}, tie = 1;
-        for (int i = 0; i < n; ++i) {
-          int cc = 0;
-          if (n_al == 2) {
-            const uint32_t d1 = adiff_u(sh.s_len[i], aln[0]), d2 = adiff_u(sh.s_len[i], aln[1]);
-            if (d1 < d2) cc = 0; else if (d1 > d2) cc = 1; else { tie = (tie + 1) % 2; cc = tie; }
+        int by_hap[2] = {0, 0};
+        if (serial) {
+          int tie = 1;
+          for (int i = 0; i < n; ++i) {
+            int cc = 0;
+            if (n_al == 2) {
+              const uint32_t d1 = adiff_u(sh.s_len[i], aln[0]), d2 = adiff_u(sh.s_len[i], aln[1]);
+              if (d1 < d2) cc = 0; else if (d1 > d2) cc = 1; else { tie = (tie + 1) % 2; cc = tie; }
+            }
+            sh.cls[i] = (int8_t)cc; by_hap[cc] += 1;
           }
-          sh.cls[i] = (int8_t)cc; by_hap[cc] += 1;
+        } else {
+          int ties = 0;
+          for (int base = 0; base < n; base += 64) {
+            const int i = base + lane;
+            int cc = 0; bool tied = false;
+            if (n_al == 2 && i < n) {
+              const uint32_t d1 = adiff_u(sh.s_len[i], aln[0]), d2 = adiff_u(sh.s_len[i], aln[1]);
+              cc = d1 > d2 ? 1 : 0; tied = d1 == d2;
+            }
+            const unsigned long long tb = __ballot(tied);
+            if (tied) cc = (ties + __popcll(tb & ((1ull << lane) - 1ull))) & 1;
+            if (i < n) sh.cls[i] = (int8_t)cc;
+            const int ones = __popcll(__ballot(i < n && cc == 1));
+            by_hap[1] += ones; by_hap[0] += (n - base < 64 ? n - base : 64) - ones;
+            ties += __popcll(tb);
+          }
         }
         auto eq_ref = [&](int al) {
           return fits ? cmp_lds(sh.bytes + sh.s_loff[rep[al]], aln[al], sh.bytes + sh.ref_off, refn) == 0 : cmp_bytes(seg_glob(rep[al]), aln[al], a.tr_blob + refo, refn) == 0;
@@ -744,7 +982,7 @@
         int order[2] = {0, 1}; int flip = 0;
         if (n_gt != 1 && !eq_ref(0) && eq_ref(1)) { order[0] = 1; order[1] = 0; flip = 1; }
         for (int oi = 0; oi < n_gt; ++oi)
-          if (aln[order[oi]] > a.allele_cap[l]) sh.bail = 1;
+          if (aln[order[oi]] > allele_cap_l) sh.bail = 1;
         sh.res_n_gt = n_gt; sh.res_flip = flip;
         for (int oi = 0; oi < n_gt; ++oi) {
           const int al = order[oi];
@@ -753,18 +991,35 @@
       }
     }
     __syncthreads();
+    GTP_MARK(GTP_CLASS);
   }
   const bool done = n > 0 && !sh.bail;
-  for (int i = lane; i < nr; i += 64) { a.classification[r0 + i] = -1; a.read_rank[r0 + i] = -1; }
-  if (n > 0 && sh.bail) { if (lane == 0) a.need_host[l] = (uint8_t)(sh.bail == 2 ? 2 : 1); return; }
-  if (!done) return;
-  __syncthreads();
+  if (serial) {
+    for (int i = lane; i < nr; i += 64) { a.classification[r0 + i] = -1; a.read_rank[r0 + i] = -1; }
+    if (n > 0 && sh.bail) { if (lane == 0) a.need_host[l] = (uint8_t)(sh.bail == 2 ? 2 : 1); return; }
+    if (!done) return;
+    __syncthreads();
+  } else {
+    int32_t* rank = reinterpret_cast<int32_t*>(sh.r_len);
+    for (int i = lane; i < nr; i += 64) rank[i] = -1;
+    __syncthreads();
+    if (done) for (int i = lane; i < n; i += 64) if (sh.s_read[i] < (uint32_t)nr) rank[sh.s_read[i]] = i;
+    __syncthreads();
+    const int flip_all = done ? sh.res_flip : 0;
+    for (int i = lane; i < nr; i += 64) {
+      const int rk = rank[i];
+      a.classification[r0 + i] = rk < 0 ? -1 : (flip_all ? 1 - sh.cls[rk] : sh.cls[rk]);
+      a.read_rank[r0 + i] = rk;
+    }
+    if (n > 0 && sh.bail) { if (lane == 0) a.need_host[l] = (uint8_t)(sh.bail == 2 ? 2 : 1); return; }
+    if (!done) return;
+  }
   const int n_gt = sh.res_n_gt;
   for (int oi = 0; oi < n_gt; ++oi) {
     const int rep = sh.res_rep[oi];
     const uint32_t len = sh.s_len[rep];
     const uint8_t* src = fits ? sh.bytes + sh.s_loff[rep] : seg_glob(rep);
-    uint8_t* dst = a.allele_blob + a.allele_off[2 * l + oi];
+    uint8_t* dst = a.allele_blob + allele_at[oi];
     for (uint32_t b = lane; b < len; b += 64) dst[b] = src[b];
     if (lane == 0) {
       a.allele_len[2 * l + oi] = len;
@@ -773,11 +1028,13 @@
       if (a.gt_size) a.gt_size[2 * l + oi] = (int32_t)len;
     }
   }
-  for (int i = lane; i < n; i += 64) {
-    a.classification[r0 + sh.s_read[i]] = sh.res_flip ? 1 - sh.cls[i] : sh.cls[i];
-    a.read_rank[r0 + sh.s_read[i]] = i;
-  }
+  if (serial)
+    for (int i = lane; i < n; i += 64) {
+      a.classification[r0 + sh.s_read[i]] = sh.res_flip ? 1 - sh.cls[i] : sh.cls[i];
+      a.read_rank[r0 + sh.s_read[i]] = i;
+    }
   if (lane == 0) { a.n_alleles[l] = n_gt; a.n_spanning_reads[l] = (uint32_t)n; a.flipped[l] = (uint8_t)sh.res_flip; }
+  GTP_MARK(GTP_OUT);
 }
 
 template <int MAXR>
diff --git a/trgt_amd/csrc/repair_queue.hpp b/trgt_amd/csrc/repair_queue.hpp
--- a/trgt_amd/csrc/repair_queue.hpp
+++ b/trgt_amd/csrc/repair_queue.hpp
@@ -12,7 +12,8 @@
 struct RepairPend {
   int32_t n_gt, n_pick; uint32_t size[2]; int32_t civ[4]; int32_t rep[2] ; int32_t grp[2] ;
 };
-enum { RC_GROUPS = 0, RC_JOBS = 1, RC_LOCI = 2, RC_FAILED = 3, RC_CIGAR = 4 , RC_OUT = 6 , RC_SCRATCH = 8 , RC_REFUSED = 10 , RC_WORDS = 16 };
+enum { RC_GROUPS = 0, RC_JOBS = 1, RC_LOCI = 2, RC_FAILED = 3, RC_CIGAR = 4 , RC_OUT = 6 , RC_SCRATCH = 8 , RC_REFUSED = 10 ,
+       RC_GT_UNSORTED = 11, RC_GT_NOFIT = 12, RC_GT_COLLISION = 13, RC_WORDS = 16 };
 struct RepairBufs {
   uint32_t* counts;
   RGroup* groups; JobDev* jobs; uint32_t* loci; RepairPend* pend;
```

Result: faster. 5.326 million loci/s (median of 6 runs) (+3.6%).
